# thu-ml/stochastic_gcn

Hardware: AMD Instinct MI355X
Metric: training edges/s (SpMM) (higher is better)
Workload: dtype f32

## Files before the change

include/sgcn.h:

```cpp
#ifndef SGCN_H
#define SGCN_H
#include <stdint.h>

#ifdef __cplusplus
extern "C" {
#endif

#define SGCN_OK 0
#define SGCN_ERR_INVALID (-1)
#define SGCN_ERR_HIP (-2)
#define SGCN_ERR_EMPTY_PROB (-3)
#define SGCN_ERR_NAN (-4)

const char* sgcn_last_error(void);
int sgcn_abi_version(void);


typedef struct { int32_t row, start, end, slot; } sgcn_seg_t;
typedef struct { int32_t row, first_slot, nslots; } sgcn_fix_t;
typedef struct {
    const sgcn_seg_t* dev_seg; int64_t nseg;
    const sgcn_fix_t* dev_fix; int64_t nfix;
    int64_t nslots;
    float* dev_ws;
// ... 59 lines not shown
                        int32_t* host_tile_rows, int32_t* host_tile_slots, sgcn_fix_t* host_fix);
void sgcn_csbuild_free(sgcn_csbuild_t* b);
int sgcn_cs_warp_table(const int32_t* host_col, int64_t nnz, int32_t K, int32_t max_buckets, int32_t mode,
                       double auto_dev, int32_t nthreads, uint32_t* host_table, int32_t* nbuckets, int32_t* shift);
int sgcn_csr_transpose_host(const int32_t* host_rowptr, const int32_t* host_col, const float* host_val, int32_t M,
                            int32_t K, int32_t nthreads, int32_t* host_t_rowptr, int32_t* host_t_col, float* host_t_val);
int32_t sgcn_host_threads(void);
int sgcn_reorder_lp(const int32_t* host_rowptr, const int32_t* host_col, int32_t n, int32_t max_iters,
                    uint32_t seed, int32_t min_size, int32_t* host_comm, int32_t* ncomm);
int sgcn_spmm_cs_f32(const sgcn_csplan_t* plan, int32_t M, int32_t K, int32_t d,
                     const float* dev_B, int64_t ldb, const int32_t* dev_gidx,
                     const float* dev_rscale, const float* dev_cscale,
                     float* dev_C, int64_t ldc, float beta, void* stream);

int sgcn_spmm_cs_variant(const sgcn_csplan_t* plan, int32_t d, char* buf, int32_t buflen);

typedef struct {
    int32_t VW, NW, RW, S, U;
    int32_t nparts;
    int32_t unit;
    int32_t xcd_tile_ptr[9];
    int64_t ntiles, nchunks, nent;
    const int32_t* dev_tile_chunk_ptr;
    const int32_t* dev_chunk_cols;
    const int32_t* dev_chunk_hdr;
    const int64_t* dev_ent_ptr;
    const uint32_t* dev_words;
    const float* dev_vals;
    const float* dev_row_fold;
    const int32_t* dev_tile_rows;
    const int32_t* dev_tile_slots;
    const sgcn_fix_t* dev_fix; int64_t nfix; int64_t nslots;
    float* dev_ws; int64_t ws_elems;
} sgcn_ldsplan_t;
typedef struct sgcn_ldsplan_host sgcn_ldsplan_host_t;
int sgcn_ldsplan_create(const int32_t* host_rowptr, const int32_t* host_col, const float* host_val,
                        int32_t M, int32_t K, const int32_t* host_col_pos, const int32_t* host_row_group,
                        int32_t VW, int32_t T, int32_t min_reuse, int32_t mode, int32_t ring_slots,
                        sgcn_ldsplan_host_t** out);
int sgcn_ldsplan_sizes(const sgcn_ldsplan_host_t* h, int64_t* sizes19);
int sgcn_ldsplan_export(const sgcn_ldsplan_host_t* h, int32_t* tile_chunk_ptr, int32_t* chunk_cols,
                        int32_t* chunk_hdr, int64_t* ent_ptr, uint32_t* words, float* vals, float* row_fold,
                        int32_t* tile_rows, int32_t* tile_slots, sgcn_fix_t* fix, int32_t* res_rowptr,
                        int32_t* res_col, float* res_val);
void sgcn_ldsplan_destroy(sgcn_ldsplan_host_t* h);
int sgcn_spmm_lds_f32(const sgcn_ldsplan_t* plan, int32_t M, int32_t K, int32_t d,
                      const float* dev_B, int64_t ldb, const float* dev_rscale,
                      float* dev_C, int64_t ldc, float beta, void* stream);

int sgcn_lds_profile_buffer(void* dev_buf);

int sgcn_tune(const char* key, int64_t value);
int64_t sgcn_tune_get(const char* key);

int sgcn_vr_aggregate_f32(const int32_t* dev_a_rowptr, const int32_t* dev_a_col,
                          const float* dev_a_val, const int32_t* dev_f_rowptr,
                          const int32_t* dev_f_col, const float* dev_f_val,
                          int32_t n1, int32_t n0, int32_t nf, int32_t d,
                          const float* dev_h, const float* dev_mu, int64_t ldx,
                          const float* dev_Hbar, int64_t ldh,
                          const int32_t* dev_ifield, const int32_t* dev_ffield,
                          const float* dev_s,
                          float* dev_out_h, float* dev_out_mu, int64_t ldo,
                          int32_t cvd, int32_t concat_self,
                          const sgcn_plan_t* f_plan ,
                          void* stream);

int sgcn_vr_aggregate_pre_f32(const int32_t* dev_f_rowptr, const int32_t* dev_f_col, const float* dev_f_val,
                              int32_t n1, int32_t nf, int32_t d, const float* dev_Hbar, int64_t ldh,
                              const int32_t* dev_ffield, float* dev_accP, const sgcn_plan_t* f_plan,
                              void* stream);
int sgcn_vr_aggregate_post_f32(const int32_t* dev_a_rowptr, const int32_t* dev_a_col, const float* dev_a_val,
                               int32_t n1, int32_t n0, int32_t d, const float* dev_h, const float* dev_mu,
                               int64_t ldx, const float* dev_Hbar, int64_t ldh, const int32_t* dev_ifield,
                               const float* dev_s, float* dev_out_h, float* dev_out_mu, int64_t ldo,
                               int32_t cvd, int32_t concat_self, const float* dev_accP, void* stream);

int sgcn_gather_rows_f32(const float* dev_in, int64_t ldi, const int32_t* dev_r, int32_t n,
                         int32_t d, float* dev_out, int64_t ldo, void* stream);

int sgcn_scatter_rows_f32(float* dev_H, int64_t ldh, const int32_t* dev_r, int32_t n,
                          int32_t d, const float* dev_src, int64_t lds, void* stream);

int sgcn_vr_aggregate_h16(const int32_t* dev_a_rowptr, const int32_t* dev_a_col,
                          const float* dev_a_val, const int32_t* dev_f_rowptr,
                          const int32_t* dev_f_col, const float* dev_f_val,
                          int32_t n1, int32_t n0, int32_t nf, int32_t d,
                          const float* dev_h, const float* dev_mu, int64_t ldx,
                          const uint16_t* dev_Hbar, int64_t ldh,
                          const int32_t* dev_ifield, const int32_t* dev_ffield,
                          const float* dev_s,
                          float* dev_out_h, float* dev_out_mu, int64_t ldo,
                          int32_t cvd, int32_t concat_self,
                          const sgcn_plan_t* f_plan, void* stream);
int sgcn_vr_aggregate_pre_h16(const int32_t* dev_f_rowptr, const int32_t* dev_f_col, const float* dev_f_val,
                              int32_t n1, int32_t nf, int32_t d, const uint16_t* dev_Hbar, int64_t ldh,
                              const int32_t* dev_ffield, float* dev_accP, const sgcn_plan_t* f_plan,
                              void* stream);
int sgcn_vr_aggregate_post_h16(const int32_t* dev_a_rowptr, const int32_t* dev_a_col, const float* dev_a_val,
                               int32_t n1, int32_t n0, int32_t d, const float* dev_h, const float* dev_mu,
                               int64_t ldx, const uint16_t* dev_Hbar, int64_t ldh, const int32_t* dev_ifield,
                               const float* dev_s, float* dev_out_h, float* dev_out_mu, int64_t ldo,
                               int32_t cvd, int32_t concat_self, const float* dev_accP, void* stream);
int sgcn_gather_rows_h16(const uint16_t* dev_H, int64_t ldh, const int32_t* dev_r, int32_t n,
                         int32_t d, float* dev_out, int64_t ldo, void* stream);
int sgcn_scatter_rows_h16(uint16_t* dev_H, int64_t ldh, const int32_t* dev_r, int32_t n,
// ... 301 lines not shown
```

stochastic_gcn_amd/_ffi.py:

```python
import ctypes as C
import os

import torch

_HERE = os.path.dirname(os.path.abspath(__file__))
LIB_PATH = os.path.join(_HERE, "libsgcn.so")

ABI_VERSION = 16

c_i32p = C.POINTER(C.c_int32)
c_f32p = C.POINTER(C.c_float)


class Seg(C.Structure):
    _fields_ = [("row", C.c_int32), ("start", C.c_int32), ("end", C.c_int32), ("slot", C.c_int32)]


class Fix(C.Structure):
    _fields_ = [("row", C.c_int32), ("first_slot", C.c_int32), ("nslots", C.c_int32)]


class CsPlan(C.Structure):
    _fields_ = [("R", C.c_int32), ("ntiles", C.c_int64), ("dev_tile_ptr", C.c_void_p),
                ("dev_colrow", C.c_void_p), ("dev_val", C.c_void_p), ("dev_tile_rows", C.c_void_p),
# ... 83 lines not shown
    "sgcn_spmm_lds_f32": (C.c_int, [C.POINTER(LdsPlan), C.c_int32, C.c_int32, C.c_int32, P, C.c_int64, P, P,
                                    C.c_int64, C.c_float, P]),
    "sgcn_vr_aggregate_f32": (C.c_int, [P, P, P, P, P, P, C.c_int32, C.c_int32, C.c_int32,
                                        C.c_int32, P, P, C.c_int64, P, C.c_int64, P, P, P, P, P,
                                        C.c_int64, C.c_int32, C.c_int32, C.POINTER(Plan), P]),
    "sgcn_vr_aggregate_pre_f32": (C.c_int, [P, P, P, C.c_int32, C.c_int32, C.c_int32, P, C.c_int64, P, P,
                                            C.POINTER(Plan), P]),
    "sgcn_vr_aggregate_post_f32": (C.c_int, [P, P, P, C.c_int32, C.c_int32, C.c_int32, P, P, C.c_int64, P, C.c_int64,
                                             P, P, P, P, C.c_int64, C.c_int32, C.c_int32, P, P]),
    "sgcn_gather_rows_f32": (C.c_int, [P, C.c_int64, P, C.c_int32, C.c_int32, P, C.c_int64, P]),
    "sgcn_scatter_rows_f32": (C.c_int, [P, C.c_int64, P, C.c_int32, C.c_int32, P, C.c_int64, P]),
    "sgcn_vr_aggregate_h16": (C.c_int, [P, P, P, P, P, P, C.c_int32, C.c_int32, C.c_int32,
                                        C.c_int32, P, P, C.c_int64, P, C.c_int64, P, P, P, P, P,
                                        C.c_int64, C.c_int32, C.c_int32, C.POINTER(Plan), P]),
    "sgcn_vr_aggregate_pre_h16": (C.c_int, [P, P, P, C.c_int32, C.c_int32, C.c_int32, P, C.c_int64, P, P,
                                            C.POINTER(Plan), P]),
    "sgcn_vr_aggregate_post_h16": (C.c_int, [P, P, P, C.c_int32, C.c_int32, C.c_int32, P, P, C.c_int64, P, C.c_int64,
                                             P, P, P, P, C.c_int64, C.c_int32, C.c_int32, P, P]),
    "sgcn_gather_rows_h16": (C.c_int, [P, C.c_int64, P, C.c_int32, C.c_int32, P, C.c_int64, P]),
    "sgcn_scatter_rows_h16": (C.c_int, [P, C.c_int64, P, C.c_int32, C.c_int32, P, C.c_int64, P]),
    "sgcn_hist_apply_h16": (C.c_int, [P, C.c_int64, P, C.c_int32, C.c_int32, C.c_int32, P, P]),
    "sgcn_spmm_csr_b16": (C.c_int, [P, P, P, C.c_int32, C.c_int32, C.c_int32, P, C.c_int64, P,
                                    P, P, P, C.c_int64, C.c_float, C.POINTER(Plan), P]),
    "sgcn_spmm_csr_add_b16": (C.c_int, [P, P, P, C.c_int32, C.c_int32, C.c_int32, P, C.c_int64, P,
                                        P, P, P, C.c_int64, C.c_float, C.POINTER(Plan), P, C.c_int64, C.c_int32, P]),
    "sgcn_spmm_cs_b16": (C.c_int, [C.POINTER(CsPlan), C.c_int32, C.c_int32, C.c_int32, P, C.c_int64, P,
                                   P, P, P, C.c_int64, C.c_float, P]),
    "sgcn_spmm_cs_variant_b16": (C.c_int, [C.POINTER(CsPlan), C.c_int32, C.c_char_p, C.c_int32]),
    "sgcn_coll_available": (C.c_int, [C.POINTER(C.c_int32)]),
    "sgcn_coll_retain": (C.c_int, []),
    "sgcn_coll_abort": (C.c_int, []),
    "sgcn_coll_async_error": (C.c_int, []),
    "sgcn_coll_unique_id": (C.c_int, [P]),
    "sgcn_coll_init": (C.c_int, [P, C.c_int32, C.c_int32]),
    "sgcn_coll_world": (C.c_int, []),
    "sgcn_coll_destroy": (C.c_int, []),
    "sgcn_coll_allreduce_avg_f32": (C.c_int, [P, C.c_int64, P]),
    "sgcn_coll_allgather_i32": (C.c_int, [P, P, C.c_int64, P]),
    "sgcn_coll_init_exchange": (C.c_int, [P]),
    "sgcn_coll_has_exchange": (C.c_int, []),
    "sgcn_coll_allgather_x_i32": (C.c_int, [P, P, C.c_int64, P]),
    "sgcn_hist_pack_f32": (C.c_int, [P, C.c_int32, P, C.c_int64, C.c_int32, C.c_int32, P, P]),
    "sgcn_hist_apply_f32": (C.c_int, [P, C.c_int64, P, C.c_int32, C.c_int32, C.c_int32, P, P]),
    "sgcn_csr_slice_indptr": (C.c_int, [C.c_int32, P, P, P]),
    "sgcn_csr_slice_indptr_dev": (C.c_int, [C.c_int32, P, P, P, P]),
    "sgcn_scale_rows_f32": (C.c_int, [P, C.c_int64, P, C.c_int32, C.c_int32, P, C.c_int64, P]),
    "sgcn_csr_slice_f32": (C.c_int, [C.c_int32, P, P, P, P, P, P, P, P, P]),
    "sgcn_ln_act_fwd_f32": (C.c_int, [P, C.c_int64, P, P, C.c_int32, C.c_int32, C.c_float, C.c_int32,
                                      P, C.c_int64, P, P, P]),
    "sgcn_ln_act_bwd_ws_floats": (C.c_int64, [C.c_int32, C.c_int32]),
    "sgcn_ln_act_bwd_f32": (C.c_int, [P, C.c_int64, P, C.c_int64, P, P, P, C.c_int32, C.c_int32,
                                      C.c_int32, P, C.c_int64, P, P, P, P]),
    "sgcn_gemm_ws_floats": (C.c_int64, [C.c_int32, C.c_int32, C.c_int32]),
    "sgcn_gemm_f32": (C.c_int, [C.c_int32, C.c_int32, C.c_int32, C.c_int32, C.c_int32, P, C.c_int64, P,
                                C.c_int64, P, C.c_int64, C.c_int32, P, P, P, P]),
    "sgcn_gemm_mb16_ws_floats": (C.c_int64, [C.c_int32, C.c_int32, C.c_int32, C.c_int32, C.c_int32]),
    "sgcn_gemm_mb16_f32": (C.c_int, [C.c_int32, C.c_int32, C.c_int32, C.c_int32, C.c_int32, P, C.c_int64, P,
                                     C.c_int64, P, C.c_int64, C.c_int32, P, P, P, P]),
    "sgcn_gemm_mb16_a16": (C.c_int, [C.c_int32, C.c_int32, C.c_int32, C.c_int32, C.c_int32, P, C.c_int64, P,
                                     C.c_int64, P, C.c_int64, C.c_int32, P, P, P, P]),
    "sgcn_dense_fwd_f32": (C.c_int, [C.c_int32, C.c_int32, C.c_int32, P, C.c_int64, P, C.c_int64, C.c_int32,
                                     P, C.c_int64, P, P, C.c_float, C.c_int32, P, C.c_int64, P, P, P, P, P, P, P]),
    "sgcn_dense_bwd_f32": (C.c_int, [C.c_int32, C.c_int32, C.c_int32, P, C.c_int64, P, C.c_int64, P, P, P,
                                     C.c_int32, P, C.c_int64, P, C.c_int64, P, C.c_int64, P, P, P, C.c_int64,
                                     P, P, P, P, P]),
    "sgcn_det_pre_f32": (C.c_int, [P, P, C.c_int64, C.c_float, P, P]),
    "sgcn_det_pre_bwd_f32": (C.c_int, [P, P, C.c_int64, C.c_float, P, P, P]),
    "sgcn_square_f32": (C.c_int, [P, C.c_int64, C.c_float, P, P]),
    "sgcn_addmul_f32": (C.c_int, [P, P, P, C.c_int64, C.c_float, P]),
    "sgcn_det_lnvar_fwd_f32": (C.c_int, [P, P, P, C.c_int32, C.c_int32, C.c_float, P, P]),
    "sgcn_det_lnvar_bwd_f32": (C.c_int, [P, P, P, P, P, C.c_int32, C.c_int32, C.c_float, P, P, P, P, P]),
    "sgcn_det_relu_fwd_f32": (C.c_int, [P, P, C.c_int64, P, P, P]),
    "sgcn_det_relu_bwd_f32": (C.c_int, [P, P, P, P, C.c_int64, P, P, P]),
    "sgcn_gauss_sample_f32": (C.c_int, [P, P, C.c_int64, C.c_uint32, P, P]),
    "sgcn_gauss_sample_bwd_f32": (C.c_int, [P, P, C.c_int64, C.c_uint32, P, P]),
    "sgcn_det_agg_prep_f32": (C.c_int, [P, P, P, P, C.c_int64, P, C.c_int32, C.c_int32, P, P, P, P, P, P]),
    "sgcn_det_agg_prep_bwd_f32": (C.c_int, [P, P, P, P, P, C.c_int32, C.c_int32, P, C.c_int64, C.c_int32, P, P]),
    "sgcn_relu_eps_f32": (C.c_int, [P, C.c_int64, C.c_int32, C.c_int32, C.c_float, P, C.c_int64, P]),
    "sgcn_gate_f32": (C.c_int, [P, C.c_int64, P, C.c_int64, C.c_int32, C.c_int32, P, P]),
    "sgcn_dropout_f32": (C.c_int, [P, C.c_int64, C.c_int32, C.c_int32, P, P, C.c_int64, P]),
    "sgcn_softmax_ce_f32": (C.c_int, [P, C.c_int64, P, C.c_int64, C.c_int32, C.c_int32, P, C.c_int64,
                                      P, C.c_int64, P, P, P]),
    "sgcn_sigmoid_ce_f32": (C.c_int, [P, C.c_int64, P, C.c_int64, C.c_int32, C.c_int32, P, C.c_int64,
                                      P, C.c_int64, P, P, P]),
    "sgcn_softmax_ce_rows_f32": (C.c_int, [P, C.c_int64, P, C.c_int64, C.c_int32, C.c_int32, P, C.c_int32, P, C.c_int64,
                                           P, C.c_int64, P, P, P]),
    "sgcn_sigmoid_ce_rows_f32": (C.c_int, [P, C.c_int64, P, C.c_int64, C.c_int32, C.c_int32, P, C.c_int32, P, C.c_int64,
                                           P, C.c_int64, P, P, P]),
    "sgcn_l2_penalty_f32": (C.c_int, [P, C.c_int64, C.c_int64, C.c_float, P, P, P]),
    "sgcn_csr_transpose_ws_ints": (C.c_int64, [C.c_int32, C.c_int64]),
    "sgcn_csr_transpose_index": (C.c_int, [C.c_int32, C.c_int64, P, P, P, P, P, P, P]),
    "sgcn_gather_f32": (C.c_int, [P, P, C.c_int64, P, P]),
    "sgcn_step_run": (C.c_int, [C.POINTER(StepOp), C.c_int32, P, C.c_int32, P]),
    "sgcn_step_fill": (C.c_int, [C.POINTER(StepFill), P, C.c_int64, C.c_int64, C.c_int64, C.c_int64, C.c_int64, C.c_float,
                                 P, C.c_int64]),
    "sgcn_copy_h2d_async": (C.c_int, [P, P, C.c_int64, P]),
    "sgcn_adam_f32": (C.c_int, [P, P, P, P, C.c_int64, C.c_float, C.c_float, C.c_float, C.c_float, P]),
    "sgcn_adam_ema_f32": (C.c_int, [P, P, P, P, P, C.c_int64, C.c_float, C.c_float, C.c_float, C.c_float, C.c_float, C.c_float, P]),
    "sgcn_moments_add_f32": (C.c_int, [P, C.c_int64, C.c_int64, P, P, P]),
    "sgcn_moments_summary_f64": (C.c_int, [P, P, C.c_int64, P, C.c_int64, P, P]),
    "sgcn_hist_error_ws_doubles": (C.c_int64, []),
    "sgcn_hist_error_f32": (C.c_int, [P, C.c_int64, P, C.c_int64, C.c_int64, C.c_int32, P, P, P]),
    "sgcn_hist_error_h16": (C.c_int, [P, C.c_int64, P, C.c_int64, C.c_int64, C.c_int32, P, P, P]),
    "sgcn_sched_create": (C.c_int, [P, P, P, C.c_int32, C.c_int32, C.c_int32, C.c_int32,
                                    C.c_int32, C.POINTER(C.c_void_p)]),
    "sgcn_sched_destroy": (None, [C.c_void_p]),
# ... 67 lines not shown
```

stochastic_gcn_amd/csrc/sgcn_agg.hip:

```cpp
#include "sgcn_dev.h"
#include <type_traits>

namespace sgcn {

int group_lanes(int nvec);

template <class HT>
struct AggArgsT {
    const int32_t* a_rowptr; const int32_t* a_col; const float* a_val;
    const int32_t* f_rowptr; const int32_t* f_col; const float* f_val;
    const sgcn_seg_t* seg; int64_t nseg; int64_t nsegblk;
    const float* h; const float* mu; int64_t ldx;
    const HT* H; int64_t ldh;
    const int32_t* ifield; const int32_t* ffield; const float* s;
    float* out_h; float* out_mu; int64_t ldo;
    int32_t d, nvec, cvd, off, concat;
    float* ws; int64_t ldw;
    int32_t pchunks;
    float* accP_out; const float* accP_in;
};


template <int VW>
__device__ __forceinline__ void store_masked(float* p, typename Vec<VW>::type v, int left) {
    if (left >= VW) vstore<VW>(p, v);
    else vstore_head<VW>(p, v, left);
}

template <int G, int VW, class HT>
__device__ __forceinline__ void agg_apart(const AggArgsT<HT>& a, int row, int vi, int lig, bool act,
                                          typename Vec<VW>::type& acc1, typename Vec<VW>::type& acc2) {
    typedef typename Vec<VW>::type VT;
    acc1 = vzero<VW>(); acc2 = vzero<VW>();
    const int start = uniform_i<G>(a.a_rowptr[row]), end = uniform_i<G>(a.a_rowptr[row + 1]);
    const int64_t voff = (int64_t)vi * VW;
    for (int p0 = start; p0 < end; p0 += G) {
        const int n = min(G, end - p0);
        int mycol = 0, myhist = 0;
        float myval = 0.f;
        if (lig < n) {
            mycol = a.a_col[p0 + lig];
            myval = a.a_val[p0 + lig];
            myhist = a.ifield[mycol];
        }
        for (int j = 0; j < n; j++) {
            const int c = bcast_i<G>(mycol, j);
            const int hr = bcast_i<G>(myhist, j);
            const float v = bcast_f<G>(myval, j);
            if (!act) continue;
            const VT hb = hload<VW>(a.H + (int64_t)hr * a.ldh + voff);
            const VT xv = vload<VW>(a.h + (int64_t)c * a.ldx + voff);
            if constexpr (VW == 1 && !std::is_same<HT, float>::value) {
                if (a.cvd) {
                    const float mv = a.mu[(int64_t)c * a.ldx + voff];
                    acc1 = __builtin_fmaf(v, mv - hb, acc1);
                    acc2 = __builtin_fmaf(v, xv - mv, acc2);
                } else {
                    acc1 = __builtin_fmaf(v, xv, acc1);
                    acc2 = __builtin_fmaf(v, hb, acc2);
                }
            } else if (a.cvd) {
                const VT mv = vload<VW>(a.mu + (int64_t)c * a.ldx + voff);
                acc1 += v * (mv - hb);
                acc2 += v * (xv - mv);
            } else {
                acc1 += v * xv;
                acc2 += v * hb;
            }
        }
    }
}

template <int VW, class HT>
__device__ __forceinline__ void agg_epilogue(const AggArgsT<HT>& a, int row, int vi, bool act, typename Vec<VW>::type accP,
                                             typename Vec<VW>::type acc1, typename Vec<VW>::type acc2) {
    typedef typename Vec<VW>::type VT;
    if (!act) return;
    const int64_t voff = (int64_t)vi * VW;
    const int left = a.d - vi * VW;
    float* oh = a.out_h + (int64_t)row * a.ldo;
    if (a.cvd) {
        float* om = a.out_mu + (int64_t)row * a.ldo;
        const VT mu_nbr = acc1 + accP;
        const VT h_nbr = acc2 * a.s[row] + mu_nbr;
        store_masked<VW>(oh + a.off + voff, h_nbr, left);
        store_masked<VW>(om + a.off + voff, mu_nbr, left);
        if (a.concat) {
            store_masked<VW>(oh + voff, vload<VW>(a.h + (int64_t)row * a.ldx + voff), left);
            store_masked<VW>(om + voff, vload<VW>(a.mu + (int64_t)row * a.ldx + voff), left);
        }
    } else {
        const VT out = (acc1 - acc2) + accP;
        store_masked<VW>(oh + a.off + voff, out, left);
        if (a.concat) store_masked<VW>(oh + voff, vload<VW>(a.h + (int64_t)row * a.ldx + voff), left);
    }
}

template <int G, int VW, class HT>
__device__ __forceinline__ void agg_finish(const AggArgsT<HT>& a, int row, int vi, int lig, bool act,
                                           typename Vec<VW>::type accP) {
    typename Vec<VW>::type acc1, acc2;
    agg_apart<G, VW>(a, row, vi, lig, act, acc1, acc2);
    agg_epilogue<VW>(a, row, vi, act, accP, acc1, acc2);
}

static int p_chunks(int32_t d, const void* Hbar, int64_t ldh, const float* ws) {
    const int vw = pick_vw(d, {Hbar, ws}, {ldh, ((int64_t)d + 3) / 4 * 4});
    return kBlock / group_lanes((d + vw - 1) / vw) - 1;
}

constexpr int agg_max_chunks(int G, int VW) { return (kBlock / G) * (4 / VW) - 1 < 31 ? (kBlock / G) * (4 / VW) - 1 : 31; }

template <int G, int VW, int U, class HT>
__global__ __launch_bounds__(kBlock) void agg_row_kernel(AggArgsT<HT> a) {
    typedef typename Vec<VW>::type VT;
    constexpr int NG = kBlock / G, NP = NG - 1;
    constexpr int NC = agg_max_chunks(G, VW);
    __shared__ float part[NC + 2][G * VW];
    const int lig = threadIdx.x & (G - 1), gq = threadIdx.x / G;
    const int slab = (int)(blockIdx.x / a.nseg);
    const int64_t s = blockIdx.x % a.nseg;
    int row, start, end, slot;
    if (a.seg) {
        const sgcn_seg_t sg = a.seg[s];
        row = sg.row; start = sg.start; end = sg.end; slot = sg.slot;
    } else {
        row = (int)s; start = a.f_rowptr[s]; end = a.f_rowptr[s + 1]; slot = -1;
    }
    row = uniform_i<G>(row); start = uniform_i<G>(start);
    end = uniform_i<G>(end); slot = uniform_i<G>(slot);
    const int vi = slab * G + lig;
    const bool act = vi < a.nvec;
    const bool finish_here = slot < 0 && !a.accP_out;
    const HT* Hl = a.H + (int64_t)vi * VW;

    const int nc = a.pchunks;
    if (gq < NP) {
        const int chunk = (end - start + nc - 1) / nc;
        for (int ck = gq; ck < nc; ck += NP) {
            const int gs = start + ck * chunk, ge = min(end, gs + chunk);
            VT accP = vzero<VW>();
            for (int p0 = gs; p0 < ge; p0 += G) {
                const int n = min(G, ge - p0);
                int myrow = 0;
                float myval = 0.f;
                if (lig < n) {
                    myrow = a.ffield[a.f_col[p0 + lig]];
                    myval = a.f_val[p0 + lig];
                }
                hpin<HT, VW>(myrow); hpin<HT, VW>(myval);
                for (int j = 0; j < n; j += U) {
                    typename HRaw<HT, VW>::type b[U];
                    float v[U];
#pragma unroll
                    for (int u = 0; u < U; u++) {
                        const bool in = j + u < n;
                        const int c = bcast_i<G>(myrow, in ? j + u : 0);
                        v[u] = in ? bcast_f<G>(myval, j + u) : 0.f;
                        b[u] = (act && in) ? hraw<VW>(Hl + (int64_t)c * a.ldh) : hraw_zero<HT, VW>();
                    }
#pragma unroll
                    for (int u = 0; u < U; u++) { hpin<HT, VW>(b[u]); accP += v[u] * hwiden<VW>(b[u]); }
                }
            }
            vstore<VW>(&part[ck][lig * VW], accP);
        }
    } else if (finish_here) {
        VT acc1, acc2;
        agg_apart<G, VW>(a, row, vi, lig, act, acc1, acc2);
        vstore<VW>(&part[NC][lig * VW], acc1);
        vstore<VW>(&part[NC + 1][lig * VW], acc2);
    }
    __syncthreads();
    if (gq != 0) return;
    VT accP = vload<VW>(&part[0][lig * VW]);
    if (nc == NP) {
#pragma unroll
        for (int q = 1; q < NP; q++) accP += vload<VW>(&part[q][lig * VW]);
    } else {
        for (int q = 1; q < nc; q++) accP += vload<VW>(&part[q][lig * VW]);
    }
    if (slot >= 0) { if (act) vstore<VW>(a.ws + (int64_t)slot * a.ldw + (int64_t)vi * VW, accP); }
    else if (a.accP_out) { if (act) vstore<VW>(a.accP_out + (int64_t)row * a.ldw + (int64_t)vi * VW, accP); }
    else agg_epilogue<VW>(a, row, vi, act, accP, vload<VW>(&part[NC][lig * VW]), vload<VW>(&part[NC + 1][lig * VW]));
}

template <int G, int VW, class HT>
__global__ __launch_bounds__(kBlock) void agg_fix_kernel(AggArgsT<HT> a, const sgcn_fix_t* fix, int64_t nfix) {
    typedef typename Vec<VW>::type VT;
    constexpr int GPB = kBlock / G;
    const int lig = threadIdx.x & (G - 1);
    const int64_t nfblk = (nfix + GPB - 1) / GPB;
    const int slab = (int)(blockIdx.x / nfblk);
    const int64_t f = (blockIdx.x % nfblk) * GPB + threadIdx.x / G;
    if (f >= nfix) return;
    const sgcn_fix_t fx = fix[f];
    const int vi = slab * G + lig;
    const bool act = vi < a.nvec;
    VT accP = vzero<VW>();
    if (act) {
        const float* w = a.ws + (int64_t)fx.first_slot * a.ldw + (int64_t)vi * VW;
        for (int q = 0; q < fx.nslots; q++) accP += vload<VW>(w + (int64_t)q * a.ldw);
    }
    if (a.accP_out) { if (act) vstore<VW>(a.accP_out + (int64_t)fx.row * a.ldw + (int64_t)vi * VW, accP); }
    else agg_finish<G, VW>(a, uniform_i<G>(fx.row), vi, lig, act, accP);
}

template <int G, int VW, class HT>
__global__ __launch_bounds__(kBlock) void agg_post_kernel(AggArgsT<HT> a, int32_t n1) {
    typedef typename Vec<VW>::type VT;
    constexpr int GPB = kBlock / G;
    const int lig = threadIdx.x & (G - 1);
    const int64_t nrblk = ((int64_t)n1 + GPB - 1) / GPB;
    const int slab = (int)(blockIdx.x / nrblk);
    const int64_t row = (blockIdx.x % nrblk) * GPB + threadIdx.x / G;
    if (row >= n1) return;
    const int vi = slab * G + lig;
    const bool act = vi < a.nvec;
    const VT accP = act ? vload<VW>(a.accP_in + row * a.ldw + (int64_t)vi * VW) : vzero<VW>();
    agg_finish<G, VW>(a, uniform_i<G>((int)row), vi, lig, act, accP);
}

template <int VW, class HT>
static int launch_agg_post(int G, const AggArgsT<HT>& a, int32_t n1, hipStream_t st) {
    const int nslab = (a.nvec + G - 1) / G;
#define SGCN_AGGP_CASE(GG)                                                                               \
    case GG: {                                                                                           \
        const int64_t nrblk = ((int64_t)n1 + (kBlock / GG) - 1) / (kBlock / GG);                          \
        hipLaunchKernelGGL((agg_post_kernel<GG, VW, HT>), dim3((unsigned)(nrblk * nslab)), dim3(kBlock), 0, st, a, n1); \
        break;                                                                                           \
    }
    switch (G) {
        SGCN_AGGP_CASE(8)
        SGCN_AGGP_CASE(16)
        SGCN_AGGP_CASE(32)
        SGCN_AGGP_CASE(64)
        default: return fail(SGCN_ERR_INVALID, "vr_aggregate_post: bad group %d", G);
    }
#undef SGCN_AGGP_CASE
    SGCN_HIP_TRY(hipGetLastError());
    return SGCN_OK;
}

template <int VW, class HT>
static int launch_agg(int G, const AggArgsT<HT>& a, const sgcn_plan_t* plan, hipStream_t st) {
    const int nslab = (a.nvec + G - 1) / G;
    SGCN_REQUIRE(a.pchunks >= 1 && a.pchunks <= agg_max_chunks(G, VW), "vr_aggregate: %d chunks of a P row, at most %d here",
                 a.pchunks, agg_max_chunks(G, VW));
    const int64_t nblocks = a.nseg * nslab;
    SGCN_REQUIRE(nblocks < (1ll << 31), "vr_aggregate: grid too large");
#define SGCN_AGG_CASE(GG)                                                                          \
    case GG: {                                                                                     \
        hipLaunchKernelGGL((agg_row_kernel<GG, VW, 16, HT>), dim3((unsigned)nblocks), dim3(kBlock), 0,  \
                           st, a);                                                                 \
        if (plan && plan->nfix > 0) {                                                              \
            const int64_t nfblk = (plan->nfix + (kBlock / GG) - 1) / (kBlock / GG);               \
            hipLaunchKernelGGL((agg_fix_kernel<GG, VW, HT>), dim3((unsigned)(nfblk * nslab)),          \
                               dim3(kBlock), 0, st, a, plan->dev_fix, plan->nfix);                 \
// ... 16 lines not shown

using namespace sgcn;

template <class HT>
static const void* vw_table(const HT* Hbar) { return std::is_same<HT, float>::value ? Hbar : nullptr; }

template <class HT>
static int vr_aggregate(const char* who, const int32_t* a_rowptr, const int32_t* a_col, const float* a_val,
                        const int32_t* f_rowptr, const int32_t* f_col, const float* f_val, int32_t n1, int32_t n0, int32_t nf,
                        int32_t d, const float* h, const float* mu, int64_t ldx, const HT* Hbar, int64_t ldh,
                        const int32_t* ifield, const int32_t* ffield, const float* s, float* out_h, float* out_mu, int64_t ldo,
                        int32_t cvd, int32_t concat_self, const sgcn_plan_t* f_plan, void* stream) {
    constexpr bool kH16 = !std::is_same<HT, float>::value;
    SGCN_REQUIRE(n1 >= 0 && n0 >= 0 && nf >= 0 && d >= 0, "%s: negative size", who);
    if constexpr (kH16) { if (int rc = h16_table_ok(who, Hbar, ldh, d)) return rc; }
    if (n1 == 0 || d == 0) return SGCN_OK;
    SGCN_REQUIRE(a_rowptr && f_rowptr && h && Hbar && ifield && out_h, "%s: null operand", who);
    SGCN_REQUIRE(nf == 0 || ffield, "%s: null ffield", who);
    SGCN_REQUIRE(!cvd || (mu && s && out_mu), "%s: cvd needs mu, s, out_mu", who);
    SGCN_REQUIRE(n1 <= n0 || !concat_self, "%s: concat_self needs n1 <= n0", who);
    const int64_t width = concat_self ? 2 * (int64_t)d : d;
    SGCN_REQUIRE(ldx >= d && ldh >= d && ldo >= width, "%s: leading dimension too small", who);

    AggArgsT<HT> a{};
    a.a_rowptr = a_rowptr; a.a_col = a_col; a.a_val = a_val;
    a.f_rowptr = f_rowptr; a.f_col = f_col; a.f_val = f_val;
    a.h = h; a.mu = mu; a.ldx = ldx; a.H = Hbar; a.ldh = ldh;
    a.ifield = ifield; a.ffield = ffield; a.s = s;
    a.out_h = out_h; a.out_mu = out_mu; a.ldo = ldo;
    a.d = d; a.cvd = cvd; a.concat = concat_self; a.off = concat_self ? d : 0;
    a.nseg = n1;
    if (f_plan) {
        SGCN_REQUIRE(f_plan->dev_seg && f_plan->nseg >= n1, "%s: malformed plan", who);
        a.seg = f_plan->dev_seg; a.nseg = f_plan->nseg;
        a.ws = f_plan->dev_ws; a.ldw = ((int64_t)d + 3) / 4 * 4;
        if (f_plan->nfix > 0) {
            SGCN_REQUIRE(f_plan->dev_fix && f_plan->dev_ws, "%s: plan needs dev_fix/dev_ws", who);
            SGCN_REQUIRE(f_plan->ws_elems >= f_plan->nslots * a.ldw, "%s: workspace too small", who);
        }
    }
    int vw = pick_vw(d, {h, mu, vw_table(Hbar), out_h, out_mu, f_plan ? f_plan->dev_ws : nullptr}, {ldx, ldh, ldo});
    if (concat_self) while (vw > 1 && d % vw != 0) vw >>= 1;
    a.nvec = (d + vw - 1) / vw;
    const int G = group_lanes(a.nvec);
    a.pchunks = p_chunks(d, vw_table(Hbar), ldh, f_plan ? f_plan->dev_ws : nullptr);
    a.nsegblk = (a.nseg + (kBlock / G) - 1) / (kBlock / G);
    hipStream_t st = (hipStream_t)stream;
    if (vw == 4) return launch_agg<4>(G, a, f_plan, st);
    if (vw == 2) return launch_agg<2>(G, a, f_plan, st);
    return launch_agg<1>(G, a, f_plan, st);
}

template <class HT>
static int vr_aggregate_pre(const char* who, const int32_t* f_rowptr, const int32_t* f_col, const float* f_val, int32_t n1,
                            int32_t nf, int32_t d, const HT* Hbar, int64_t ldh, const int32_t* ffield, float* accP,
                            const sgcn_plan_t* f_plan, void* stream) {
    constexpr bool kH16 = !std::is_same<HT, float>::value;
    SGCN_REQUIRE(n1 >= 0 && nf >= 0 && d >= 0, "%s: negative size", who);
    if constexpr (kH16) { if (int rc = h16_table_ok(who, Hbar, ldh, d)) return rc; }
    if (n1 == 0 || d == 0) return SGCN_OK;
    SGCN_REQUIRE(f_rowptr && Hbar && accP && ldh >= d, "%s: bad operand", who);
    SGCN_REQUIRE(nf == 0 || ffield, "%s: null ffield", who);
    AggArgsT<HT> a{};
    a.f_rowptr = f_rowptr; a.f_col = f_col; a.f_val = f_val;
    a.H = Hbar; a.ldh = ldh; a.ffield = ffield; a.d = d;
    a.ldw = ((int64_t)d + 3) / 4 * 4;
    a.accP_out = accP;
    a.nseg = n1;
    if (f_plan) {
        SGCN_REQUIRE(f_plan->dev_seg && f_plan->nseg >= n1, "%s: malformed plan", who);
        a.seg = f_plan->dev_seg; a.nseg = f_plan->nseg; a.ws = f_plan->dev_ws;
        if (f_plan->nfix > 0) {
            SGCN_REQUIRE(f_plan->dev_fix && f_plan->dev_ws, "%s: plan needs dev_fix/dev_ws", who);
            SGCN_REQUIRE(f_plan->ws_elems >= f_plan->nslots * a.ldw, "%s: workspace too small", who);
        }
    }
    const int vw = pick_vw(d, {vw_table(Hbar), accP, f_plan ? f_plan->dev_ws : nullptr}, {ldh, a.ldw});
    a.nvec = (d + vw - 1) / vw;
    const int G = group_lanes(a.nvec);
    a.pchunks = p_chunks(d, vw_table(Hbar), ldh, f_plan ? f_plan->dev_ws : nullptr);
    a.nsegblk = (a.nseg + (kBlock / G) - 1) / (kBlock / G);
    hipStream_t st = (hipStream_t)stream;
    if (vw == 4) return launch_agg<4>(G, a, f_plan, st);
    if (vw == 2) return launch_agg<2>(G, a, f_plan, st);
    return launch_agg<1>(G, a, f_plan, st);
}

template <class HT>
static int vr_aggregate_post(const char* who, const int32_t* a_rowptr, const int32_t* a_col, const float* a_val, int32_t n1,
                             int32_t n0, int32_t d, const float* h, const float* mu, int64_t ldx, const HT* Hbar, int64_t ldh,
                             const int32_t* ifield, const float* s, float* out_h, float* out_mu, int64_t ldo, int32_t cvd,
                             int32_t concat_self, const float* accP, void* stream) {
    constexpr bool kH16 = !std::is_same<HT, float>::value;
    SGCN_REQUIRE(n1 >= 0 && n0 >= 0 && d >= 0, "%s: negative size", who);
    if constexpr (kH16) { if (int rc = h16_table_ok(who, Hbar, ldh, d)) return rc; }
    if (n1 == 0 || d == 0) return SGCN_OK;
    SGCN_REQUIRE(a_rowptr && h && Hbar && ifield && out_h && accP, "%s: null operand", who);
    SGCN_REQUIRE(!cvd || (mu && s && out_mu), "%s: cvd needs mu, s, out_mu", who);
    SGCN_REQUIRE(n1 <= n0 || !concat_self, "%s: concat_self needs n1 <= n0", who);
    const int64_t width = concat_self ? 2 * (int64_t)d : d;
    SGCN_REQUIRE(ldx >= d && ldh >= d && ldo >= width, "%s: leading dimension too small", who);
    AggArgsT<HT> a{};
    a.a_rowptr = a_rowptr; a.a_col = a_col; a.a_val = a_val;
    a.h = h; a.mu = mu; a.ldx = ldx; a.H = Hbar; a.ldh = ldh; a.ifield = ifield; a.s = s;
    a.out_h = out_h; a.out_mu = out_mu; a.ldo = ldo;
    a.d = d; a.cvd = cvd; a.concat = concat_self; a.off = concat_self ? d : 0;
    a.ldw = ((int64_t)d + 3) / 4 * 4;
    a.accP_in = accP;
    int vw = pick_vw(d, {h, mu, vw_table(Hbar), out_h, out_mu, accP}, {ldx, ldh, ldo, a.ldw});
    if (concat_self) while (vw > 1 && d % vw != 0) vw >>= 1;
    a.nvec = (d + vw - 1) / vw;
    const int G = group_lanes(a.nvec);
    hipStream_t st = (hipStream_t)stream;
    if (vw == 4) return launch_agg_post<4>(G, a, n1, st);
    if (vw == 2) return launch_agg_post<2>(G, a, n1, st);
    return launch_agg_post<1>(G, a, n1, st);
}

extern "C" int sgcn_vr_aggregate_f32(const int32_t* a_rowptr, const int32_t* a_col, const float* a_val,
                                     const int32_t* f_rowptr, const int32_t* f_col, const float* f_val, int32_t n1,
                                     int32_t n0, int32_t nf, int32_t d, const float* h, const float* mu, int64_t ldx,
                                     const float* Hbar, int64_t ldh, const int32_t* ifield, const int32_t* ffield,
                                     const float* s, float* out_h, float* out_mu, int64_t ldo, int32_t cvd,
                                     int32_t concat_self, const sgcn_plan_t* f_plan, void* stream) {
    return vr_aggregate<float>("vr_aggregate", a_rowptr, a_col, a_val, f_rowptr, f_col, f_val, n1, n0, nf, d, h, mu, ldx, Hbar,
                               ldh, ifield, ffield, s, out_h, out_mu, ldo, cvd, concat_self, f_plan, stream);
}

extern "C" int sgcn_vr_aggregate_pre_f32(const int32_t* f_rowptr, const int32_t* f_col, const float* f_val, int32_t n1,
                                         int32_t nf, int32_t d, const float* Hbar, int64_t ldh, const int32_t* ffield,
                                         float* accP, const sgcn_plan_t* f_plan, void* stream) {
    return vr_aggregate_pre<float>("vr_aggregate_pre", f_rowptr, f_col, f_val, n1, nf, d, Hbar, ldh, ffield, accP, f_plan, stream);
}

extern "C" int sgcn_vr_aggregate_post_f32(const int32_t* a_rowptr, const int32_t* a_col, const float* a_val, int32_t n1,
                                          int32_t n0, int32_t d, const float* h, const float* mu, int64_t ldx,
                                          const float* Hbar, int64_t ldh, const int32_t* ifield, const float* s,
                                          float* out_h, float* out_mu, int64_t ldo, int32_t cvd, int32_t concat_self,
                                          const float* accP, void* stream) {
// ... 30 lines not shown
```

stochastic_gcn_amd/csrc/sgcn_fuse.h:

```cpp
#pragma once
#include <cstdint>
#include "../../include/sgcn.h"

namespace sgcn {

struct CeLastLayer {
    const float* W = nullptr; int64_t ldw = 0; int32_t K = 0;
    float* dx = nullptr; int64_t lddx = 0; const sgcn_dropout_t* dx_drop = nullptr;
    const float* hx = nullptr; int64_t ldhx = 0; int32_t kg = 1; const sgcn_dropout_t* h_drop = nullptr;
    bool pre = false;
    const float* px = nullptr; int64_t ldpx = 0; int32_t PK = 0; const float* PW = nullptr;
    int32_t pS = 1, pkchunk = 0, pkg = 1; const sgcn_dropout_t* p_drop = nullptr;
    const float* poff = nullptr; const float* psc = nullptr; float peps = 0.f; int32_t prelu = 0;
    float* pY = nullptr; int64_t ldpy = 0; float* pxhat = nullptr; float* prstd = nullptr;
};

}
```

stochastic_gcn_amd/csrc/sgcn_gemm.hip:

```cpp
#include "sgcn_dev.h"
#include "sgcn_bwd.h"

namespace sgcn {

typedef float f16acc __attribute__((ext_vector_type(16)));

constexpr int kTM = 32, kTN = 128, kTK = 32;

struct GemmArgs {
    const float* A; int64_t lda;
    const float* B; int64_t ldb;
    float* C; int64_t ldc;
    int32_t M, N, K;
    int32_t accumulate;
    int32_t kchunk;
    float* ws;
    const float* offset; const float* scale; float eps; int32_t relu;
    float* xhat; float* rstd;
    int32_t epi;
    const float* A2; int64_t lda2; int32_t a_split;
    DropArgs drop_a;
    DropArgs drop_c;
    int32_t vec_a, vec_b;
    const int32_t* a_gidx;
    const int32_t* a_gidx2;
};

__device__ __forceinline__ float wsum(float v) {
#pragma unroll
    for (int o = 32; o > 0; o >>= 1) v += __shfl_xor(v, o, 64);
    return v;
}

constexpr int kAsFloats = kTM * (kTK + 1), kBsFloats = kTK * (kTN + 4);
constexpr int kGroupFloats = kAsFloats + kBsFloats;

template <bool TA, bool TB, int KG>
__device__ __forceinline__ void gemm_body(const GemmArgs& g, const int bx, const int by, const int bz) {
    extern __shared__ float smem[];
    const int kg = threadIdx.x / kBlock;
    const int tid = threadIdx.x % kBlock, lane = tid & 63, wave = tid >> 6;
    float (*As)[kTK + 1] = reinterpret_cast<float (*)[kTK + 1]>(smem + kg * kGroupFloats);
    float (*Bs)[kTN + 4] = reinterpret_cast<float (*)[kTN + 4]>(smem + kg * kGroupFloats + kAsFloats);
    const int m0 = bx * kTM, n0 = by * kTN;
    const int kbeg = bz * g.kchunk;
    const int kend = min(g.K, kbeg + g.kchunk);
    f16acc acc = {};
    float ra[4], rb[16];
    float ep_scale[2] = {1.f, 1.f}, ep_offset[2] = {0.f, 0.f};
    if (g.epi == 2) {
#pragma unroll
        for (int e = 0; e < 2; e++) {
            const int c = (threadIdx.x & 63) + e * kWave;
            if (c < g.N) { ep_scale[e] = g.scale[c]; ep_offset[e] = g.offset[c]; }
// ... 121 lines not shown
#pragma unroll
        for (int r = 0; r < 16; r++) {
            const int row = m0 + (r & 3) + 8 * (r >> 2) + 4 * (lane >> 5), col = n0 + cj;
            if (row < g.M && col < g.N) {
                float* p = base + (int64_t)row * ld + col;
                float v = acc[r];
                if (g.drop_c.on) v *= drop_factor(g.drop_c, row, col);
                *p = add ? *p + v : v;
            }
        }
        return;
    }
    float (*Cs)[kTN + 4] = reinterpret_cast<float (*)[kTN + 4]>(smem + kAsFloats);
    if (KG > 1) __syncthreads();
    if (kg == 0) {
#pragma unroll
        for (int r = 0; r < 16; r++) Cs[(r & 3) + 8 * (r >> 2) + 4 * (lane >> 5)][cj] = acc[r];
    }
    __syncthreads();
    for (int rr = kg * (kBlock / kWave) + wave; rr < kTM; rr += KG * (kBlock / kWave)) {
        const int row = m0 + rr;
        if (row >= g.M) break;
        float* yr = g.C + (int64_t)row * g.ldc;
        if (g.epi == 1) {
            for (int c = lane; c < g.N; c += kWave) { const float v = Cs[rr][c]; yr[c] = g.relu ? fmaxf(v, 0.f) : v; }
            continue;
        }
        float s = 0.f;
        for (int c = lane; c < g.N; c += kWave) s += Cs[rr][c];
        const float mean = wsum(s) / (float)g.N;
        float q = 0.f;
        for (int c = lane; c < g.N; c += kWave) { const float t = Cs[rr][c] - mean; q += t * t; }
        const float rs = rsqrtf(wsum(q) / (float)g.N + g.eps);
        if (lane == 0) g.rstd[row] = rs;
        float* hr = g.xhat + (int64_t)row * g.N;
#pragma unroll
        for (int e = 0; e < 2; e++) {
            const int c = lane + e * kWave;
            if (c < g.N) {
                const float h = (Cs[rr][c] - mean) * rs;
                hr[c] = h;
                const float v = h * ep_scale[e] + ep_offset[e];
                yr[c] = g.relu ? fmaxf(v, 0.f) : v;
            }
        }
    }
}

template <bool TA, bool TB, int KG>
__global__ __launch_bounds__(kBlock * KG) void gemm_kernel(GemmArgs g) {
    gemm_body<TA, TB, KG>(g, (int)blockIdx.x, (int)blockIdx.y, (int)blockIdx.z);
}

struct GemmGroup {
    GemmArgs g[kMaxGroup];
    int32_t first[kMaxGroup + 1];
    int32_t gx[kMaxGroup], gy[kMaxGroup];
    int32_t n;
};

template <bool TA, bool TB, int KG>
__global__ __launch_bounds__(kBlock * KG) void gemm_group_kernel(GemmGroup G) {
    const int b = (int)blockIdx.x;
    int j = 0;
#pragma unroll
    for (int q = 1; q < kMaxGroup; q++) j += (q < G.n && b >= G.first[q]) ? 1 : 0;
    const int l = b - G.first[j];
    const int gx = G.gx[j], gy = G.gy[j];
    gemm_body<TA, TB, KG>(G.g[j], l % gx, (l / gx) % gy, l / (gx * gy));
}

__global__ void splitk_reduce_kernel(const float* __restrict__ ws, int32_t S, int32_t M, int32_t N,
                                     float* __restrict__ C, int64_t ldc, int32_t accumulate) {
    const int64_t i = (int64_t)blockIdx.x * blockDim.x + threadIdx.x;
    const int64_t mn = (int64_t)M * N;
    if (i >= mn) return;
    float s = 0.f;
    for (int z = 0; z < S; z++) s += ws[(int64_t)z * mn + i];
    float* p = C + (i / N) * ldc + (i % N);
    *p = accumulate ? *p + s : s;
}

__global__ void dense_bwd_reduce_kernel(ReduceJob j, int32_t gemm_blocks, const float* __restrict__ ln_partial,
                                        int32_t nblk, int32_t d, float* __restrict__ doffset,
                                        float* __restrict__ dscale, int32_t ln_accumulate) {
    if ((int)blockIdx.x < gemm_blocks) {
        const int64_t i = (int64_t)blockIdx.x * blockDim.x + threadIdx.x;
        const int64_t mn = (int64_t)j.M * j.N;
        if (i >= mn) return;
        float s = 0.f;
        for (int z = 0; z < j.S; z++) s += j.ws[(int64_t)z * mn + i];
        float* p = j.C + (i / j.N) * j.ldc + (i % j.N);
        *p = j.accumulate ? *p + s : s;
    } else {
        ln_param_reduce_cols32(ln_partial, nblk, d, doffset, dscale, (int)blockIdx.x - gemm_blocks, ln_accumulate != 0);
    }
}

__global__ void dense_bwd_reduce_multi_kernel(ReduceMulti R) { reduce_multi_body(R, (int)blockIdx.x, nullptr); }

__global__ __launch_bounds__(kBlock) void splitk_ln_act_kernel(const float* __restrict__ ws, int32_t S,
                                                               GemmArgs g) {
    const int lane = threadIdx.x & 63;
    const int64_t row = (int64_t)blockIdx.x * (kBlock / kWave) + threadIdx.x / kWave;
    if (row >= g.M) return;
    const int64_t mn = (int64_t)g.M * g.N;
    float v[2];
    float sc[2] = {1.f, 1.f}, of[2] = {0.f, 0.f};
    if (g.epi == 2) {
#pragma unroll
        for (int e = 0; e < 2; e++) {
            const int c = lane + e * kWave;
            if (c < g.N) { sc[e] = g.scale[c]; of[e] = g.offset[c]; }
        }
    }
#pragma unroll
    for (int e = 0; e < 2; e++) {
        const int c = lane + e * kWave;
        float s = 0.f;
        if (c < g.N)
            for (int z = 0; z < S; z++) s += ws[(int64_t)z * mn + row * g.N + c];
        v[e] = s;
    }
    float* yr = g.C + row * g.ldc;
    if (g.epi == 2) {
        const float mean = wsum(v[0] + v[1]) / (float)g.N;
        float q = 0.f;
#pragma unroll
        for (int e = 0; e < 2; e++) if (lane + e * kWave < g.N) { const float t = v[e] - mean; q += t * t; }
        const float rs = rsqrtf(wsum(q) / (float)g.N + g.eps);
        if (lane == 0) g.rstd[row] = rs;
#pragma unroll
        for (int e = 0; e < 2; e++) {
            const int c = lane + e * kWave;
            if (c < g.N) {
                const float h = (v[e] - mean) * rs;
                g.xhat[row * g.N + c] = h;
                const float y = h * sc[e] + of[e];
                yr[c] = g.relu ? fmaxf(y, 0.f) : y;
            }
        }
    } else {
#pragma unroll
        for (int e = 0; e < 2; e++) {
            const int c = lane + e * kWave;
            if (c < g.N) yr[c] = (g.epi == 1 && g.relu) ? fmaxf(v[e], 0.f) : v[e];
        }
    }
}


struct RowDense {
    const float* W; int64_t ldw; int32_t N, kg;
    const float* offset; const float* scale; float eps; int32_t relu, epi;
    DropArgs drop;
    float* Y; int64_t ldy; float* xhat; float* rstd;
};

__global__ __launch_bounds__(kBlock) void splitk_ln_dense_kernel(const float* __restrict__ ws, int32_t S, GemmArgs g, RowDense d) {
    extern __shared__ __attribute__((aligned(1024))) float wl[];
    const int lane = threadIdx.x & 63;
    const int64_t row = (int64_t)blockIdx.x * (kBlock / kWave) + threadIdx.x / kWave;
    const bool live = row < g.M;
    const int K2 = g.N, total = K2 * d.N;
    {
        const int total4 = total / 4, wave = threadIdx.x >> 6;
        for (int base4 = wave * kWave; base4 < total4; base4 += (kBlock / kWave) * kWave) {
            const int i4 = min(base4 + lane, total4 - 1);
            __builtin_amdgcn_global_load_lds((const __attribute__((address_space(1))) void*)(d.W + (int64_t)i4 * 4),
                                             (__attribute__((address_space(3))) void*)(wl + (int64_t)base4 * 4), 16, 0, 0);
        }
    }
    float sc1[2] = {1.f, 1.f}, of1[2] = {0.f, 0.f}, sc2[2] = {1.f, 1.f}, of2[2] = {0.f, 0.f};
#pragma unroll
    for (int e = 0; e < 2; e++) {
        const int c = lane + e * kWave;
        if (g.epi == 2 && c < g.N) { sc1[e] = g.scale[c]; of1[e] = g.offset[c]; }
        if (d.epi == 2 && c < d.N) { sc2[e] = d.scale[c]; of2[e] = d.offset[c]; }
    }
    const int64_t mn = (int64_t)g.M * g.N;
    float v[2] = {0.f, 0.f};
    if (live) {
#pragma unroll
        for (int e = 0; e < 2; e++) {
            const int c = lane + e * kWave;
            float s = 0.f;
            if (c < g.N)
                for (int z = 0; z < S; z++) s += ws[(int64_t)z * mn + row * g.N + c];
            v[e] = s;
        }
    }
    asm volatile("s_waitcnt vmcnt(0)" ::: "memory");
    __syncthreads();
    if (!live) return;
    float x[2];
    float* yr = g.C + row * g.ldc;
    if (g.epi == 2) {
        const float mean = wsum(v[0] + v[1]) / (float)g.N;
        float q = 0.f;
#pragma unroll
        for (int e = 0; e < 2; e++) if (lane + e * kWave < g.N) { const float t = v[e] - mean; q += t * t; }
        const float rs = rsqrtf(wsum(q) / (float)g.N + g.eps);
        if (lane == 0) g.rstd[row] = rs;
#pragma unroll
        for (int e = 0; e < 2; e++) {
            const int c = lane + e * kWave;
            x[e] = 0.f;
            if (c < g.N) {
                const float h = (v[e] - mean) * rs;
                g.xhat[row * g.N + c] = h;
                const float y = h * sc1[e] + of1[e];
                x[e] = g.relu ? fmaxf(y, 0.f) : y;
// ... 16 lines not shown
        const float xs = s0 < 2 ? x[0] : x[1];
        const int kb = s0 * 32, lb = kb & (kWave - 1);
        const float* wk = wl + kb * d.N;
        float p0 = a0[gi], p1 = a1[gi];
        if (kb + 32 <= K2) {
#pragma unroll
            for (int q = 0; q < 4; q++) {
                float w0[8], w1[8];
#pragma unroll
                for (int u = 0; u < 8; u++) { w0[u] = wk[(q * 8 + u) * d.N + c0]; w1[u] = wk[(q * 8 + u) * d.N + c1]; }
#pragma unroll
                for (int u = 0; u < 8; u++) {
                    const float xv = __int_as_float(__builtin_amdgcn_readlane(__float_as_int(xs), lb + q * 8 + u));
                    p0 = fmaf(xv, w0[u], p0); p1 = fmaf(xv, w1[u], p1);
                }
            }
        } else {
            for (int kk = 0; kb + kk < K2; kk++) {
                const float xv = __int_as_float(__builtin_amdgcn_readlane(__float_as_int(xs), lb + kk));
                p0 = fmaf(xv, wk[kk * d.N + c0], p0); p1 = fmaf(xv, wk[kk * d.N + c1], p1);
            }
        }
        a0[gi] = p0; a1[gi] = p1;
    }
    const float z[2] = {d.kg > 1 ? a0[0] + a0[1] : a0[0], d.kg > 1 ? a1[0] + a1[1] : a1[0]};
    float* y2 = d.Y + row * d.ldy;
    if (d.epi != 2) {
#pragma unroll
        for (int e = 0; e < 2; e++) {
            const int c = lane + e * kWave;
            if (c < d.N) y2[c] = (d.epi == 1 && d.relu) ? fmaxf(z[e], 0.f) : z[e];
        }
        return;
    }
    float s = 0.f;
#pragma unroll
    for (int e = 0; e < 2; e++) if (lane + e * kWave < d.N) s += z[e];
    const float mean = wsum(s) / (float)d.N;
    float q = 0.f;
#pragma unroll
    for (int e = 0; e < 2; e++) if (lane + e * kWave < d.N) { const float t = z[e] - mean; q += t * t; }
    const float rs = rsqrtf(wsum(q) / (float)d.N + d.eps);
    if (lane == 0) d.rstd[row] = rs;
#pragma unroll
    for (int e = 0; e < 2; e++) {
        const int c = lane + e * kWave;
        if (c < d.N) {
            const float h = (z[e] - mean) * rs;
            d.xhat[row * d.N + c] = h;
            const float y = h * sc2[e] + of2[e];
            y2[c] = d.relu ? fmaxf(y, 0.f) : y;
        }
    }
}

}

using namespace sgcn;

static int split_factor(int M, int N, int K) {
    const int tiles = ((M + kTM - 1) / kTM) * ((N + kTN - 1) / kTN);
    int s = 256 / std::max(tiles, 1);
    const int min_steps = tune_get("gemm_min_steps") > 0 ? tune_get("gemm_min_steps") : 3;
    s = std::min(s, K / (min_steps * kTK));
    return std::max(s, 1);
}

template <bool TA, bool TB, int KG>
static void launch_one(const GemmArgs& g, dim3 grid, hipStream_t st) {
    const size_t lds = (size_t)KG * kGroupFloats * sizeof(float);
    static bool raised = false;
    if (lds > 64 * 1024 && !raised) {
        (void)hipFuncSetAttribute(reinterpret_cast<const void*>(&gemm_kernel<TA, TB, KG>),
                                  hipFuncAttributeMaxDynamicSharedMemorySize, (int)lds);
        raised = true;
    }
    hipLaunchKernelGGL((gemm_kernel<TA, TB, KG>), grid, dim3(kBlock * KG), lds, st, g);
}

template <bool TA, bool TB>
static void launch_kg(const GemmArgs& g, dim3 grid, int kgroups, hipStream_t st) {
    if (kgroups >= 4) launch_one<TA, TB, 4>(g, grid, st);
    else if (kgroups == 2) launch_one<TA, TB, 2>(g, grid, st);
    else launch_one<TA, TB, 1>(g, grid, st);
}

struct GemmPlan { dim3 grid; int kgroups, S, epi; };

static GemmPlan prepare_gemm(GemmArgs& g, float* ws, int ta = 0, int tb = 0) {
    auto al = [](const void* p, int64_t ld) { return p && ((uintptr_t)p % 16 == 0) && (ld % 4 == 0); };
    g.vec_a = al(g.A, g.lda) && (!g.A2 || al(g.A2, g.lda2)) && (ta ? g.M : g.K) % 4 == 0;
    g.vec_b = al(g.B, g.ldb) && (tb ? g.K : g.N) % 4 == 0;
    int S = ws ? split_factor(g.M, g.N, g.K) : 1;
    g.kchunk = ((g.K + S - 1) / S + kTK - 1) / kTK * kTK;
    S = g.K > 0 ? (g.K + g.kchunk - 1) / g.kchunk : 1;
    if (g.K == 0) g.kchunk = kTK;
    g.ws = S > 1 ? ws : nullptr;
    GemmPlan p;
    p.epi = g.epi;
    p.S = S;
    if (S > 1) g.epi = 0;
    p.grid = dim3((unsigned)((g.M + kTM - 1) / kTM), (unsigned)((g.N + kTN - 1) / kTN), (unsigned)S);
    const int steps = (std::min(g.kchunk, g.K) + kTK - 1) / kTK;
    const int blocks = (int)(p.grid.x * p.grid.y * p.grid.z);
    p.kgroups = (blocks <= 128 && steps >= 8) ? 4 : ((blocks <= 256 && steps >= 4) ? 2 : 1);
    return p;
}

namespace sgcn {
void gemm_fwd_shape(int M, int N, int K, int* S, int* kgroups, int* kchunk) {
    GemmArgs g{};
    g.M = M; g.N = N; g.K = K;
    float dummy;
    const GemmPlan p = prepare_gemm(g, sgcn_gemm_ws_floats(M, N, K) > 0 ? &dummy : nullptr);
    *S = p.S; *kgroups = p.kgroups;
    if (kchunk) *kchunk = g.kchunk;
}
}

static void launch_prepared(const GemmArgs& g, const GemmPlan& p, int ta, int tb, hipStream_t st) {
    if (!ta && !tb) launch_kg<false, false>(g, p.grid, p.kgroups, st);
    else if (ta && !tb) launch_kg<true, false>(g, p.grid, p.kgroups, st);
    else if (!ta && tb) launch_kg<false, true>(g, p.grid, p.kgroups, st);
    else launch_kg<true, true>(g, p.grid, p.kgroups, st);
}

static int launch_gemm(GemmArgs g, int ta, int tb, float* ws, hipStream_t st, ReduceJob* defer = nullptr) {
    if (defer) defer->pending = 0;
    const GemmPlan p = prepare_gemm(g, ws, ta, tb);
    const int S = p.S, epi = p.epi;
    launch_prepared(g, p, ta, tb, st);
    if (S > 1 && epi != 0) {
        g.epi = epi;
        const unsigned rb = (unsigned)((g.M + (kBlock / kWave) - 1) / (kBlock / kWave));
        hipLaunchKernelGGL(splitk_ln_act_kernel, dim3(rb), dim3(kBlock), 0, st, g.ws, S, g);
    } else if (S > 1 && defer) {
        *defer = ReduceJob{g.ws, S, g.M, g.N, g.C, g.ldc, g.accumulate, 1};
    } else if (S > 1) {
        const int64_t mn = (int64_t)g.M * g.N;
        hipLaunchKernelGGL(splitk_reduce_kernel, dim3((unsigned)((mn + 255) / 256)), dim3(256), 0, st,
                           g.ws, S, g.M, g.N, g.C, g.ldc, g.accumulate);
    }
    SGCN_HIP_TRY(hipGetLastError());
    return SGCN_OK;
}

extern "C" int64_t sgcn_gemm_ws_floats(int32_t M, int32_t N, int32_t K) {
    if (M <= 0 || N <= 0 || K <= 0) return 0;
    const int S = split_factor(M, N, K);
    return S > 1 ? (int64_t)S * M * N : 0;
}

extern "C" int sgcn_gemm_f32(int32_t trans_a, int32_t trans_b, int32_t M, int32_t N, int32_t K,
                             const float* A, int64_t lda, const float* B, int64_t ldb, float* C,
                             int64_t ldc, int32_t accumulate, float* ws,
                             const sgcn_dropout_t* drop_a, const sgcn_dropout_t* drop_c, void* stream) {
    SGCN_REQUIRE(M >= 0 && N >= 0 && K >= 0, "gemm: negative size");
    if (M == 0 || N == 0) return SGCN_OK;
    SGCN_REQUIRE(C && (K == 0 || (A && B)), "gemm: null operand");
    GemmArgs g{};
    g.A = A; g.lda = lda; g.B = B; g.ldb = ldb; g.C = C; g.ldc = ldc;
    g.M = M; g.N = N; g.K = K; g.accumulate = accumulate; g.epi = 0;
    g.drop_a = drop_args(drop_a);
    g.drop_c = drop_args(drop_c);
    SGCN_REQUIRE(!g.drop_a.on || g.drop_a.width == (trans_a ? M : K), "gemm: drop_a width must be the stored A's row length");
    SGCN_REQUIRE(!g.drop_c.on || g.drop_c.width == N, "gemm: drop_c width must be N");
    if (g.drop_c.on) ws = nullptr;
    return launch_gemm(g, trans_a, trans_b, ws, (hipStream_t)stream);
}


namespace sgcn {
int dense_fwd_pair(int32_t M, int32_t N, int32_t K, const float* X, int64_t ldx, const float* X2, int64_t ldx2, int32_t split,
                   const float* W, int64_t ldw, const float* offset, const float* scale, float eps, int32_t relu, float* Y,
                   int64_t ldy, float* xhat, float* rstd, const sgcn_dropout_t* drop, float* ws, const int32_t* gidx,
                   const int32_t* gidx2, int32_t N2, const float* W2, int64_t ldw2, const float* offset2, const float* scale2,
                   float eps2, int32_t relu2, float* Y2, int64_t ldy2, float* xhat2, float* rstd2, const sgcn_dropout_t* drop2,
                   void* stream, int* fused) {
    *fused = 0;
    if (M <= 0 || N <= 0 || N > kTN || N2 <= 0 || N2 > kTN || !ws || !W2 || !Y2 || ldw2 != N2 || ldy != N) return SGCN_OK;
    const int norm = (offset && scale) ? 1 : 0, norm2 = (offset2 && scale2) ? 1 : 0;
    if ((norm && !(xhat && rstd)) || (norm2 && !(xhat2 && rstd2))) return SGCN_OK;
    GemmArgs g{};
    g.A = X; g.lda = ldx; g.B = W; g.ldb = ldw; g.C = Y; g.ldc = ldy;
    g.M = M; g.N = N; g.K = K; g.offset = offset; g.scale = scale; g.eps = eps; g.relu = relu;
    g.xhat = xhat; g.rstd = rstd; g.epi = norm ? 2 : (relu ? 1 : 0);
    g.A2 = X2; g.lda2 = ldx2; g.a_split = split;
    g.a_gidx = gidx; g.a_gidx2 = gidx2;
    g.drop_a = drop_args(drop);
    const GemmPlan p = prepare_gemm(g, ws);
    int S2 = 0, kg2 = 0;
    gemm_fwd_shape(M, N2, N, &S2, &kg2, nullptr);
    if (p.S <= 1 || S2 != 1 || kg2 > 2 || (size_t)N * N2 * sizeof(float) > 64 * 1024 || (N * N2) % 4 || !aligned16(W2)) return SGCN_OK;
    SGCN_REQUIRE(!g.drop_a.on || g.drop_a.width == K, "dense_fwd: dropout width must be K");
    RowDense d{};
    d.W = W2; d.ldw = ldw2; d.N = N2; d.kg = kg2; d.offset = offset2; d.scale = scale2; d.eps = eps2; d.relu = relu2;
    d.epi = norm2 ? 2 : (relu2 ? 1 : 0);
    d.drop = drop_args(drop2);
    SGCN_REQUIRE(!d.drop.on || d.drop.width == N, "dense_fwd: the second layer's dropout width must be its input width");
    d.Y = Y2; d.ldy = ldy2; d.xhat = xhat2; d.rstd = rstd2;
    hipStream_t st = (hipStream_t)stream;
    launch_prepared(g, p, 0, 0, st);
    g.epi = p.epi;
    const unsigned rb = (unsigned)((g.M + (kBlock / kWave) - 1) / (kBlock / kWave));
    hipLaunchKernelGGL(splitk_ln_dense_kernel, dim3(rb), dim3(kBlock), ((size_t)N * N2 + 255) / 256 * 256 * sizeof(float), st, g.ws, p.S, g, d);
    SGCN_HIP_TRY(hipGetLastError());
    *fused = 1;
    return SGCN_OK;
}
}

extern "C" int sgcn_dense_fwd_f32(int32_t M, int32_t N, int32_t K, const float* X, int64_t ldx,
                                  const float* X2, int64_t ldx2, int32_t split,
                                  const float* W, int64_t ldw, const float* offset,
                                  const float* scale, float eps, int32_t relu, float* Y, int64_t ldy,
                                  float* xhat, float* rstd, const sgcn_dropout_t* drop, float* ws,
                                  const int32_t* gidx, const int32_t* gidx2, void* stream) {
    SGCN_REQUIRE(M >= 0 && N >= 0 && K >= 0, "dense_fwd: negative size");
    if (M == 0 || N == 0) return SGCN_OK;
    SGCN_REQUIRE((X || (X2 && split == 0)) && W && Y, "dense_fwd: null operand");
    const int norm = (offset && scale) ? 1 : 0;
    SGCN_REQUIRE(!norm || (xhat && rstd), "dense_fwd: LayerNorm needs xhat / rstd");
    SGCN_REQUIRE(N <= kTN || (!norm && !relu), "dense_fwd: fused epilogue needs N <= 128");
    GemmArgs g{};
    g.A = X; g.lda = ldx; g.B = W; g.ldb = ldw; g.C = Y; g.ldc = ldy;
    g.M = M; g.N = N; g.K = K; g.offset = offset; g.scale = scale; g.eps = eps; g.relu = relu;
    g.xhat = xhat; g.rstd = rstd; g.epi = norm ? 2 : (relu ? 1 : 0);
    SGCN_REQUIRE(!X2 || (split >= 0 && split <= M), "dense_fwd: bad split");
    g.A2 = X2; g.lda2 = ldx2; g.a_split = split;
    g.a_gidx = gidx; g.a_gidx2 = gidx2;
    g.drop_a = drop_args(drop);
    SGCN_REQUIRE(!g.drop_a.on || g.drop_a.width == K, "dense_fwd: dropout width must be K");
    return launch_gemm(g, 0, 0, N <= kTN ? ws : nullptr, (hipStream_t)stream);
}


namespace sgcn {
namespace {
struct AuxCtx {
    hipStream_t st = nullptr;
    hipEvent_t fork = nullptr, join = nullptr;
    float* ring = nullptr;
    int64_t cap = 0, off = 0, want = 0;
    bool pending = false;
};
AuxCtx& aux_ctx() { static AuxCtx c; return c; }
int g_dw_recorded = 0;
int g_grad_store = 0;

int aux_init(AuxCtx& c) {
    if (c.st) return SGCN_OK;
    SGCN_HIP_TRY(hipStreamCreateWithFlags(&c.st, hipStreamNonBlocking));
    SGCN_HIP_TRY(hipEventCreateWithFlags(&c.fork, hipEventDisableTiming));
    SGCN_HIP_TRY(hipEventCreateWithFlags(&c.join, hipEventDisableTiming));
    return SGCN_OK;
}
}

int aux_fork(void* stream, void** aux_stream) {
// ... 300 lines not shown
```

stochastic_gcn_amd/csrc/sgcn_spmm.hip:

```cpp
#include "sgcn_dev.h"
#include <cstring>

namespace sgcn {

namespace {
int g_tune_nv = 0;
int g_tune_unroll = 0;
int g_tune_slabmajor = 1;
int g_tune_cs_round = 0;
int g_tune_cs_unroll = 0;
int g_tune_cs_pace = 0;
int g_tune_cs_slack = 0;
int g_tune_cs_noextra = 0;
int g_tune_step_overlap = 1;
int g_tune_step_fuse = 127;
int g_tune_cs_g2_wide = 0;
int g_tune_cs_nowarp = 0;
int g_tune_cs_last_pct = 80;
int g_tune_gemm_min_steps = 0;
int g_tune_gemm_mb16_slice_k = 0;
int g_tune_lds_wave_bias = 100;
int g_tune_lds_mix = 1;
int g_tune_lds_dbg = 0;
thread_local int tl_step_overlap = -1, tl_step_fuse = -1;
}

void step_mode_override(int overlap, int fuse) { tl_step_overlap = overlap; tl_step_fuse = fuse; }

int tune_get(const char* key) {
    if (!strcmp(key, "spmm_nv")) return g_tune_nv;
    if (!strcmp(key, "spmm_unroll")) return g_tune_unroll;
    if (!strcmp(key, "spmm_slabmajor")) return g_tune_slabmajor;
    if (!strcmp(key, "cs_round")) return g_tune_cs_round;
    if (!strcmp(key, "cs_unroll")) return g_tune_cs_unroll;
    if (!strcmp(key, "cs_pace")) return g_tune_cs_pace;
    if (!strcmp(key, "cs_slack")) return g_tune_cs_slack;
    if (!strcmp(key, "cs_noextra")) return g_tune_cs_noextra;
    if (!strcmp(key, "step_overlap")) return tl_step_overlap >= 0 ? tl_step_overlap : g_tune_step_overlap;
    if (!strcmp(key, "step_fuse")) return tl_step_fuse >= 0 ? tl_step_fuse : g_tune_step_fuse;
    if (!strcmp(key, "cs_g2_wide")) return g_tune_cs_g2_wide;
    if (!strcmp(key, "cs_nowarp")) return g_tune_cs_nowarp;
    if (!strcmp(key, "cs_last_pct")) return g_tune_cs_last_pct;
    if (!strcmp(key, "gemm_min_steps")) return g_tune_gemm_min_steps;
    if (!strcmp(key, "gemm_mb16_slice_k")) return g_tune_gemm_mb16_slice_k;
    if (!strcmp(key, "lds_wave_bias")) return g_tune_lds_wave_bias;
    if (!strcmp(key, "lds_mix")) return g_tune_lds_mix;
    if (!strcmp(key, "lds_dbg")) return g_tune_lds_dbg;
    return -1;
}

struct SpmmArgs {
    const int32_t* rowptr;
    const int32_t* col;
    const float* val;
    const sgcn_seg_t* seg;
    int64_t nseg;
    int64_t nsegblk;
    const void* B;
    int64_t ldb;
    const int32_t* gidx;
    const float* rscale;
    const float* cscale;
    float* C;
    int64_t ldc;
    float beta;
    int32_t d;
    int32_t nvec;
    float* ws;
    int64_t ldw;
    int32_t slabmajor;
    const float* add;
    int64_t ldadd;
    int32_t add_rows;
};

template <int VW>
__device__ __forceinline__ void epilogue_store(const SpmmArgs& a, int row, int vi,
                                               typename Vec<VW>::type acc, float rs) {
    float* out = a.C + (int64_t)row * a.ldc + (int64_t)vi * VW;
    typename Vec<VW>::type r = acc * rs;
    const int left = a.d - vi * VW;
    if (a.beta != 0.f) {
        if (left >= VW) r += a.beta * vload<VW>(out);
        else {
#pragma unroll
            for (int e = 0; e < VW; e++)
                if (e < left) {
                    if constexpr (VW == 1) r += a.beta * out[0]; else r[e] += a.beta * out[e];
                }
        }
    }
    if (a.add && row < a.add_rows) {
// ... 132 lines not shown
template <int VW, int U, class BT>
static bool dispatch_gnv(int G, int NV, const SpmmArgs& a, int64_t nblocks, hipStream_t st) {
    switch (G) {
        case 8: launch_seg<8, 1, VW, U, BT>(a, nblocks, st); return true;
        case 16: launch_seg<16, 1, VW, U, BT>(a, nblocks, st); return true;
        case 32: launch_seg<32, 1, VW, U, BT>(a, nblocks, st); return true;
        case 64:
            switch (NV) {
                case 1: launch_seg<64, 1, VW, U, BT>(a, nblocks, st); return true;
                case 2: launch_seg<64, 2, VW, U, BT>(a, nblocks, st); return true;
                case 3: launch_seg<64, 3, VW, U, BT>(a, nblocks, st); return true;
                case 4: launch_seg<64, 4, VW, U, BT>(a, nblocks, st); return true;
            }
    }
    return false;
}

template <int VW, class BT>
static bool dispatch_u(int U, int G, int NV, const SpmmArgs& a, int64_t nblocks, hipStream_t st) {
    switch (U) {
        case 2: return dispatch_gnv<VW, 2, BT>(G, NV, a, nblocks, st);
        case 4: return dispatch_gnv<VW, 4, BT>(G, NV, a, nblocks, st);
        case 8: return dispatch_gnv<VW, 8, BT>(G, NV, a, nblocks, st);
    }
    return false;
}

int group_lanes(int nvec) {
    if (nvec <= 8) return 8;
    if (nvec <= 16) return 16;
    if (nvec <= 32) return 32;
    return 64;
}

}

using namespace sgcn;

extern "C" int64_t sgcn_tune_get(const char* key) { return key ? tune_get(key) : -1; }

extern "C" int sgcn_tune(const char* key, int64_t value) {
    if (!key) return fail(SGCN_ERR_INVALID, "sgcn_tune: null key");
    if (!strcmp(key, "spmm_nv")) { SGCN_REQUIRE(value >= 0 && value <= 4, "spmm_nv in 0..4"); g_tune_nv = (int)value; return SGCN_OK; }
    if (!strcmp(key, "spmm_unroll")) {
        SGCN_REQUIRE(value == 0 || value == 2 || value == 4 || value == 8, "spmm_unroll in {0,2,4,8}");
        g_tune_unroll = (int)value; return SGCN_OK;
    }
    if (!strcmp(key, "spmm_slabmajor")) { g_tune_slabmajor = value != 0; return SGCN_OK; }
    if (!strcmp(key, "cs_pace")) { SGCN_REQUIRE(value >= 0, "cs_pace >= 0"); g_tune_cs_pace = (int)value; return SGCN_OK; }
    if (!strcmp(key, "cs_slack")) { SGCN_REQUIRE(value >= 0, "cs_slack >= 0"); g_tune_cs_slack = (int)value; return SGCN_OK; }
    if (!strcmp(key, "cs_noextra")) { g_tune_cs_noextra = value != 0; return SGCN_OK; }
    if (!strcmp(key, "step_overlap")) { g_tune_step_overlap = value != 0; return SGCN_OK; }
    if (!strcmp(key, "step_fuse")) { SGCN_REQUIRE(value >= 0 && value <= 127, "step_fuse in 0..127"); g_tune_step_fuse = (int)value; return SGCN_OK; }
    if (!strcmp(key, "cs_g2_wide")) { g_tune_cs_g2_wide = value != 0; return SGCN_OK; }
    if (!strcmp(key, "cs_nowarp")) { g_tune_cs_nowarp = value != 0; return SGCN_OK; }
    if (!strcmp(key, "gemm_min_steps")) { g_tune_gemm_min_steps = (int)value; return SGCN_OK; }
    if (!strcmp(key, "gemm_mb16_slice_k")) {
        SGCN_REQUIRE(value >= 0 && value <= 0x7fffffff, "gemm_mb16_slice_k >= 0");
        g_tune_gemm_mb16_slice_k = (int)value; return SGCN_OK;
    }
    if (!strcmp(key, "lds_wave_bias")) { SGCN_REQUIRE(value >= 50 && value <= 300, "lds_wave_bias in 50..300 (per cent)"); g_tune_lds_wave_bias = (int)value; return SGCN_OK; }
    if (!strcmp(key, "lds_mix")) { g_tune_lds_mix = value != 0; return SGCN_OK; }
    if (!strcmp(key, "lds_dbg")) { g_tune_lds_dbg = (int)value; return SGCN_OK; }
    if (!strcmp(key, "cs_last_pct")) { SGCN_REQUIRE(value >= 0 && value <= 100, "cs_last_pct in [0, 100]"); g_tune_cs_last_pct = (int)value; return SGCN_OK; }
    if (!strcmp(key, "cs_round")) { SGCN_REQUIRE(value >= 0, "cs_round >= 0"); g_tune_cs_round = (int)value; return SGCN_OK; }
    if (!strcmp(key, "cs_unroll")) {
        SGCN_REQUIRE(value == 0 || value == 4 || value == 8, "cs_unroll in {0,4,8}");
        g_tune_cs_unroll = (int)value; return SGCN_OK;
    }
    return fail(SGCN_ERR_INVALID, "sgcn_tune: unknown key '%s'", key);
}

template <class BT>
static int spmm_csr_add(const int32_t* rowptr, const int32_t* col, const float* val,
                        int32_t M, int32_t K, int32_t d, const BT* B, int64_t ldb,
                        const int32_t* gidx, const float* rscale, const float* cscale,
                        float* C, int64_t ldc, float beta, const sgcn_plan_t* plan,
                        const float* add, int64_t ldadd, int32_t add_rows, void* stream) {
    constexpr bool kB16 = !std::is_same<BT, float>::value;
    SGCN_REQUIRE(M >= 0 && K >= 0 && d >= 0, "spmm: negative size");
    if (M == 0 || d == 0) return SGCN_OK;
    SGCN_REQUIRE(rowptr && C && (B || K == 0), "spmm: null operand");
    SGCN_REQUIRE(ldb >= d && ldc >= d, "spmm: leading dimension smaller than d");
    if (kB16) {
        SGCN_REQUIRE(ldb % 8 == 0, "spmm: a bfloat16 operand needs ldb %% 8 == 0 (ldb %lld, d %d)", (long long)ldb, d);
        SGCN_REQUIRE(aligned16(B), "spmm: a bfloat16 operand needs a 16-byte aligned base");
    }
    hipStream_t st = (hipStream_t)stream;

    SpmmArgs a{};
    a.rowptr = rowptr; a.col = col; a.val = val;
    a.B = B; a.ldb = ldb; a.gidx = gidx; a.rscale = rscale; a.cscale = cscale;
    a.C = C; a.ldc = ldc; a.beta = beta; a.d = d;
    a.nseg = M;
    a.slabmajor = g_tune_slabmajor;
    if (add && add_rows > 0) {
        SGCN_REQUIRE(ldadd >= d && add_rows <= M, "spmm: bad addend");
        a.add = add; a.ldadd = ldadd; a.add_rows = add_rows;
    }
    if (plan) {
        SGCN_REQUIRE(plan->dev_seg && plan->nseg >= M, "spmm: malformed plan");
        a.seg = plan->dev_seg; a.nseg = plan->nseg;
        a.ws = plan->dev_ws; a.ldw = ((int64_t)d + 3) / 4 * 4;
        if (plan->nfix > 0) {
            SGCN_REQUIRE(plan->dev_fix && plan->dev_ws, "spmm: plan with split rows needs dev_fix/dev_ws");
            SGCN_REQUIRE(plan->ws_elems >= plan->nslots * a.ldw,
// ... 76 lines not shown
```

stochastic_gcn_amd/csrc/sgcn_step.cpp:

```cpp
#include <hip/hip_runtime_api.h>

#include <algorithm>
#include <chrono>
#include <cstdio>
#include <cstdlib>
#include <cstring>
#include <mutex>

#include "sgcn_host.h"
#include "sgcn_fuse.h"
#include "sgcn_bwd.h"
#include "../../include/sgcn.h"

namespace sgcn {
int dense_bwd_overlapped(int32_t n, int32_t N, int32_t K, const float* dy, int64_t lddy, const float* y, int64_t ldy,
                         const float* xhat, const float* rstd, const float* scale, int32_t relu, const float* x,
                         int64_t ldx, const float* W, int64_t ldw, float* dW, int64_t lddw, float* doffset,
                         float* dscale, float* dx, int64_t lddx, const sgcn_dropout_t* drop, float* g_tmp, float* ws,
                         const int32_t* gidx, void* stream);
int aux_join(void* stream);
void step_mode_override(int overlap, int fuse);
int dense_bwd_chain(const DenseBwdArgs& up, const DenseBwdArgs& lo, void* stream);
int aux_fork(void* stream, void** aux_stream);
int spin_launch(void* stream, int64_t usec);
int dw_group_begin();
int dw_group_flush(void* stream, bool park_reduce);
int reduce_flush(void* stream);
void dw_group_abort();
void grad_store_mode(int on);
void stats_defer(int on);
int stats_flush(void* stream);
int adam_with_stats(float* theta, const float* grad, float* m, float* v, int64_t n, float lr_t, float beta1, float beta2,
                    float eps, float* avg, float decay, float one_minus, void* stream);
bool scatter_park(float* H, int64_t ldh, const int32_t* idx, int32_t n, int32_t d, const float* src, int64_t lds);
int ce_impl(bool softmax, const float* logits, int64_t ldz, const float* labels, int64_t ldl, int32_t n, int32_t c,
            float* dlogits, int64_t lddz, float* pred, int64_t ldp, float* stats, float* rowstat, void* stream, bool overlap,
            const CeLastLayer* last);
void gemm_fwd_shape(int M, int N, int K, int* S, int* kgroups, int* kchunk);
int dense_fwd_pair(int32_t M, int32_t N, int32_t K, const float* X, int64_t ldx, const float* X2, int64_t ldx2, int32_t split,
                   const float* W, int64_t ldw, const float* offset, const float* scale, float eps, int32_t relu, float* Y,
                   int64_t ldy, float* xhat, float* rstd, const sgcn_dropout_t* drop, float* ws, const int32_t* gidx,
                   const int32_t* gidx2, int32_t N2, const float* W2, int64_t ldw2, const float* offset2, const float* scale2,
                   float eps2, int32_t relu2, float* Y2, int64_t ldy2, float* xhat2, float* rstd2, const sgcn_dropout_t* drop2,
                   void* stream, int* fused);
}

namespace {

inline float f32(int64_t v) {
    const uint32_t b = (uint32_t)(uint64_t)v;
    float f;
    std::memcpy(&f, &b, 4);
    return f;
}
template <class T> inline T* ptr(int64_t v) { return reinterpret_cast<T*>((uintptr_t)v); }

struct Args {
    int64_t v[SGCN_STEP_MAX_ARGS];
    int n, pos;
    int64_t next() { return pos < n ? v[pos++] : 0; }
    template <class T> T* p() { return ptr<T>(next()); }
    int32_t i() { return (int32_t)next(); }
    float f() { return f32(next()); }
    const sgcn_dropout_t* drop(sgcn_dropout_t* st) {
        const int64_t on = next();
        st->key = (uint32_t)next(); st->keep = f(); st->rows = i(); st->width = i();
        return on ? st : nullptr;
    }
    const sgcn_plan_t* plan(sgcn_plan_t* st) {
        const int64_t on = next();
        st->dev_seg = p<const sgcn_seg_t>(); st->nseg = next();
        st->dev_fix = p<const sgcn_fix_t>(); st->nfix = next();
        st->nslots = next(); st->dev_ws = p<float>(); st->ws_elems = next();
        if (st->nfix == 0) st->dev_fix = nullptr;
        return on ? st : nullptr;
    }
};


struct DenseFwdOp {
    int32_t M, N, K, split, relu; float eps;
    const float *X, *X2, *W, *off, *sc; int64_t ldx, ldx2, ldw, ldy, ws_cap;
    float *Y, *xhat, *rstd, *ws; const int32_t *g1, *g2;
    sgcn_dropout_t dr; bool has_drop;
    void read(Args& a) {
        M = a.i(); N = a.i(); K = a.i();
        X = a.p<const float>(); ldx = a.next(); X2 = a.p<const float>(); ldx2 = a.next(); split = a.i();
        W = a.p<const float>(); ldw = a.next(); off = a.p<const float>(); sc = a.p<const float>();
        eps = a.f(); relu = a.i();
        Y = a.p<float>(); ldy = a.next(); xhat = a.p<float>(); rstd = a.p<float>();
        has_drop = a.drop(&dr) != nullptr;
        ws = a.p<float>(); ws_cap = a.next(); g1 = a.p<const int32_t>(); g2 = a.p<const int32_t>();
    }
    const sgcn_dropout_t* drop() const { return has_drop ? &dr : nullptr; }
    bool plain() const { return !off && !sc && !relu; }
};
struct DenseBwdOp {
    int32_t n, N, K, relu;
    const float *dy, *y, *xhat, *rstd, *sc, *x, *W; int64_t lddy, ldy, ldx, ldw, lddw, lddx, ws_cap;
    float *dW, *doff, *dsc, *dx, *gtmp, *ws; const int32_t* gidx;
    sgcn_dropout_t dr; bool has_drop;
    void read(Args& a) {
        n = a.i(); N = a.i(); K = a.i();
        dy = a.p<const float>(); lddy = a.next(); y = a.p<const float>(); ldy = a.next();
        xhat = a.p<const float>(); rstd = a.p<const float>(); sc = a.p<const float>(); relu = a.i();
        x = a.p<const float>(); ldx = a.next(); W = a.p<const float>(); ldw = a.next();
        dW = a.p<float>(); lddw = a.next(); doff = a.p<float>(); dsc = a.p<float>();
        dx = a.p<float>(); lddx = a.next();
        has_drop = a.drop(&dr) != nullptr;
        gtmp = a.p<float>(); ws = a.p<float>(); ws_cap = a.next(); gidx = a.p<const int32_t>();
    }
    const sgcn_dropout_t* drop() const { return has_drop ? &dr : nullptr; }
};
struct CeOp {
    const float *z, *lab; int64_t ldz, ldl, lddz, ldp; int32_t n, c; float *dz, *pred, *stats, *rowstat;
    void read(Args& a) {
        z = a.p<const float>(); ldz = a.next(); lab = a.p<const float>(); ldl = a.next(); n = a.i(); c = a.i();
        dz = a.p<float>(); lddz = a.next(); pred = a.p<float>(); ldp = a.next(); stats = a.p<float>(); rowstat = a.p<float>();
    }
};
inline bool is_adam(int32_t op) { return op == SGCN_OP_ADAM || op == SGCN_OP_ADAM_EMA; }
constexpr int32_t f32_op(int32_t op) {
    return op == SGCN_OP_VR_AGG_H16 ? SGCN_OP_VR_AGG : op == SGCN_OP_VR_AGG_PRE_H16 ? SGCN_OP_VR_AGG_PRE
         : op == SGCN_OP_VR_AGG_POST_H16 ? SGCN_OP_VR_AGG_POST : op == SGCN_OP_SCATTER_ROWS_H16 ? SGCN_OP_SCATTER_ROWS
         : op == SGCN_OP_AUX_SCATTER_ROWS_H16 ? SGCN_OP_AUX_SCATTER_ROWS : op == SGCN_OP_HIST_APPLY_H16 ? SGCN_OP_HIST_APPLY : op;
}
inline bool is_ce(int32_t op) { return op == SGCN_OP_SOFTMAX_CE || op == SGCN_OP_SIGMOID_CE; }

}

extern "C" int sgcn_step_fill(const sgcn_step_fill_t* f, const int64_t* meta, int64_t meta_len, int64_t ip, int64_t fp,
                              int64_t seed, int64_t step, float lr, int64_t* slots, int64_t nslots) {
    if (!f || !meta || !slots || meta_len < 0 || nslots < 0 || f->n < 0 || f->n_cap < 0 || f->n_ws < 0 || f->n_keys < 0 ||
        f->n > nslots || f->lr_slot < 0 || f->lr_slot >= nslots || (f->n > 0 && (!f->idx || !f->mul || !f->base)) ||
        (f->n_cap > 0 && (!f->cap_idx || !f->cap_max)) || (f->n_ws > 0 && (!f->ws_idx || !f->ws_ld)) ||
        (f->n_keys > 0 && (!f->key_slot || !f->key_layer)))
        return sgcn::fail(SGCN_ERR_INVALID, "step_fill: bad argument");
    auto in_meta = [&](int64_t i) { return i >= 0 && i < meta_len; };
    for (int64_t j = 0; j < f->n_cap; j++) {
        if (!in_meta(f->cap_idx[j])) return sgcn::fail(SGCN_ERR_INVALID, "step_fill: capacity check outside the descriptor table");
        if (meta[f->cap_idx[j]] > f->cap_max[j]) return 1;
    }
    for (int64_t j = 0; j < f->n_ws; j++) {
        if (!in_meta(f->ws_idx[j])) return sgcn::fail(SGCN_ERR_INVALID, "step_fill: workspace check outside the descriptor table");
        if (meta[f->ws_idx[j]] * f->ws_ld[j] > f->ws_floats) return 1;
    }
    for (int64_t i = 0; i < f->n; i++)
        if (!in_meta(f->idx[i])) return sgcn::fail(SGCN_ERR_INVALID, "step_fill: slot %lld reads outside the descriptor table", (long long)i);
    for (int64_t j = 0; j < f->n_keys; j++)
        if (f->key_slot[j] < 0 || f->key_slot[j] >= nslots) return sgcn::fail(SGCN_ERR_INVALID, "step_fill: key slot out of range");
    for (int64_t i = 0; i < f->n; i++)
        slots[i] = meta[f->idx[i]] * f->mul[i] + (f->base[i] == 1 ? ip : f->base[i] == 2 ? fp : 0);
    auto fmix32 = [](uint32_t h) { h ^= h >> 16; h *= 0x85EBCA6Bu; h ^= h >> 13; h *= 0xC2B2AE35u; h ^= h >> 16; return h; };
    for (int64_t j = 0; j < f->n_keys; j++) {
        const uint32_t site = fmix32((uint32_t)seed * 0x9E3779B1u + (uint32_t)f->key_layer[j] * 0x85EBCA77u + 0x27D4EB2Fu);
        slots[f->key_slot[j]] = (int64_t)fmix32(site + (uint32_t)step * 0xC2B2AE3Du);
    }
    uint32_t bits;
    memcpy(&bits, &lr, sizeof(bits));
    slots[f->lr_slot] = (int64_t)bits;
    return SGCN_OK;
}

extern "C" int sgcn_copy_h2d_async(void* dst, const void* src, int64_t bytes, void* stream) {
    if (bytes < 0 || (bytes > 0 && (!dst || !src))) return sgcn::fail(SGCN_ERR_INVALID, "copy_h2d_async: bad argument");
    if (bytes == 0) return SGCN_OK;
// ... 41 lines not shown
        }
        SGCN_XCHG_TRY(hipStreamSynchronize((hipStream_t)stream));
        SGCN_XCHG_TRY(hipStreamSynchronize(cand[n]));
    }
    for (int i = 0; i < n; i++)
        if (i != got) (void)hipStreamDestroy(cand[i]);
    (void)hipEventDestroy(ev);
    c.st = got >= 0 ? cand[got] : nullptr;
    if (getenv("SGCN_XCHG_DEBUG")) fprintf(stderr, "sgcn: exchange stream: candidate %d of %d runs beside the step's stream\n", got, n);
    return SGCN_OK;
}

int xchg_fork(void* stream, void** side) {
    XchgCtx& c = xchg_ctx();
    if (!c.tried) {
        const int rc = xchg_pick(stream, c);
        if (rc != SGCN_OK) return rc;
        const unsigned flags = hipEventDisableTiming | (getenv("SGCN_XCHG_SYSFENCE") ? 0u : hipEventDisableSystemFence);
        SGCN_XCHG_TRY(hipEventCreateWithFlags(&c.fork, flags));
        SGCN_XCHG_TRY(hipEventCreateWithFlags(&c.done, flags));
    }
    if (!c.st) { *side = stream; return SGCN_OK; }
    if (!c.pending) {
        static const char* skip = getenv("SGCN_XCHG_DROPS_A_DEPENDENCY") ? getenv("SGCN_XCHG_SKIP") : nullptr;
        if (!(skip && strstr(skip, "fork"))) {
            SGCN_XCHG_TRY(hipEventRecord(c.fork, (hipStream_t)stream));
            SGCN_XCHG_TRY(hipStreamWaitEvent(c.st, c.fork, 0));
        }
        c.pending = true;
    }
    *side = (void*)c.st;
    return SGCN_OK;
}

int xchg_join(void* stream) {
    XchgCtx& c = xchg_ctx();
    if (!c.pending) return SGCN_OK;
    c.pending = false;
    static const char* skip = getenv("SGCN_XCHG_DROPS_A_DEPENDENCY") ? getenv("SGCN_XCHG_SKIP") : nullptr;
    if (skip && strstr(skip, "join")) return SGCN_OK;
    SGCN_XCHG_TRY(hipEventRecord(c.done, c.st));
    SGCN_XCHG_TRY(hipStreamWaitEvent((hipStream_t)stream, c.done, 0));
    return SGCN_OK;
}
}

extern "C" int sgcn_step_run(const sgcn_step_op_t* ops, int32_t nops, const int64_t* slots, int32_t nslots,
                             void* stream) {
    if (nops < 0 || (nops > 0 && !ops) || nslots < 0 || (nslots > 0 && !slots))
        return sgcn::fail(SGCN_ERR_INVALID, "step_run: bad argument");
    static std::mutex run_mutex;
    std::lock_guard<std::mutex> run_lock(run_mutex);
    bool memset_on_aux = false;
    int64_t run_overlap = sgcn_tune_get("step_overlap"), run_fuse = sgcn_tune_get("step_fuse");
    bool own_mode = false;
    for (int32_t k = 0; k < nops; k++)
        if (ops[k].op == SGCN_OP_MODE && ops[k].nargs >= 1) {
            own_mode = true;
            run_overlap = ops[k].add[0] != 0;
            if (ops[k].nargs >= 2 && ops[k].add[1] >= 0) run_fuse = ops[k].add[1] & 127;
        }
    const bool overlap = run_overlap != 0;
    const int fuse = (int)run_fuse;
    struct ModeGuard {
        bool on;
        ~ModeGuard() { if (on) sgcn::step_mode_override(-1, -1); }
    } mode{own_mode};
    if (own_mode) sgcn::step_mode_override(overlap ? 1 : 0, fuse);
    bool grouped = false, store = false, l2 = false;
    int ce_at = -1, adam_at = -1;
    for (int32_t k = 0; k < nops; k++) {
        grouped = grouped || ops[k].op == SGCN_OP_DW_FLUSH;
        store = store || ops[k].op == SGCN_OP_GRAD_STORE;
        l2 = l2 || ops[k].op == SGCN_OP_L2_PENALTY;
        if (ops[k].op == SGCN_OP_SOFTMAX_CE || ops[k].op == SGCN_OP_SIGMOID_CE) ce_at = k;
        if (is_adam(ops[k].op)) adam_at = k;
    }
    const bool park_stats = store && ce_at >= 0 && adam_at > ce_at && !l2;
    if (grouped) sgcn::dw_group_begin();
    sgcn::grad_store_mode(store ? 1 : 0);
    sgcn::stats_defer(park_stats ? 1 : 0);
    struct Guard {
        bool on; void* st;
        ~Guard() { if (on) sgcn::dw_group_abort(); sgcn::grad_store_mode(0); sgcn::stats_defer(0); sgcn::reduce_flush(st); sgcn::stats_flush(st); }
    } guard{grouped, stream};
    auto eval_args = [&](const sgcn_step_op_t& o, Args& a) {
        a.n = o.nargs; a.pos = 0;
        for (int j = 0; j < o.nargs; j++) {
            const int32_t s = o.slot[j];
            if (s >= nslots) return false;
            a.v[j] = (s < 0 ? 0 : o.mul[j] * slots[s]) + o.add[j];
        }
        return true;
    };
    int32_t skip_until = 0, dx_done_at = -1;
    struct Head { bool on = false, pre = false; int32_t at = -1, kg = 1, pS = 1, pkchunk = 0, pkg = 1; DenseFwdOp f, p; } head;
    auto peek = [&](int32_t j, Args& b) {
        return j < nops && ops[j].nargs >= 0 && ops[j].nargs <= SGCN_STEP_MAX_ARGS && eval_args(ops[j], b);
    };
    for (int32_t k = 0; k < nops; k++) {
        const sgcn_step_op_t& op = ops[k];
        if (op.nargs < 0 || op.nargs > SGCN_STEP_MAX_ARGS)
            return sgcn::fail(SGCN_ERR_INVALID, "step_run: op %d has %d arguments", k, op.nargs);
        if (k < skip_until) continue;
        Args a;
        if (!eval_args(ops[k], a)) return sgcn::fail(SGCN_ERR_INVALID, "step_run: op %d reads a slot beyond %d", k, nslots);
        int rc = SGCN_OK;
        sgcn_dropout_t dr;
        sgcn_plan_t pl;
        const int32_t base = f32_op(op.op);
        const bool h16 = base != op.op;
        if (is_adam(op.op) || base == SGCN_OP_L2_PENALTY || base == SGCN_OP_SCATTER_ROWS || base == SGCN_OP_MEMSET0 ||
            base == SGCN_OP_VR_AGG_POST || (base == SGCN_OP_DENSE_BWD && memset_on_aux)) {
            rc = sgcn::aux_join(stream);
            if (rc != SGCN_OK) return rc;
            memset_on_aux = false;
        }
        void* side = stream;
        if (overlap && (base == SGCN_OP_VR_AGG_PRE || base == SGCN_OP_AUX_SCATTER_ROWS || base == SGCN_OP_AUX_MEMSET0)) {
            rc = sgcn::aux_fork(stream, &side);
            if (rc != SGCN_OK) return rc;
        }
        auto fork_to = [&](int64_t where) {
            return where == 0 ? (int)SGCN_OK : where == 2 ? xchg_fork(stream, &side) : sgcn::aux_fork(stream, &side);
        };
        switch (op.op) {
        case SGCN_OP_DENSE_FWD: {
            DenseFwdOp f;
            f.read(a);
            head.on = false;
            Args b;
            if ((fuse & 1) && f.plain() && !f.X2 && !f.g1 && f.N <= 64 && f.K <= 128 && (int64_t)f.K * f.N * 4 <= 48 * 1024 &&
                peek(k + 1, b) && is_ce(ops[k + 1].op)) {
                CeOp ce;
                ce.read(b);
                int S = 0, kgq = 0;
                sgcn::gemm_fwd_shape(f.M, f.N, f.K, &S, &kgq, nullptr);
                if (S == 1 && kgq <= 2 && ce.z == f.Y && ce.ldz == f.ldy && ce.n == f.M && ce.c == f.N) {
                    head.on = true; head.pre = false; head.at = k + 1; head.kg = kgq; head.f = f;
                    break;
                }
            }
            if ((fuse & 16) && (fuse & 1) && !f.X2 && !f.g1 && f.N <= 128 && f.K <= 256 && (f.K * f.N) % 4 == 0 &&
                peek(k + 1, b) && ops[k + 1].op == SGCN_OP_DENSE_FWD && k + 2 < nops && is_ce(ops[k + 2].op)) {
                DenseFwdOp q;
                q.read(b);
                Args c3;
                CeOp ce;
                int S = 0, kgq = 0, S0 = 0, kg0 = 0, kc0 = 0;
                sgcn::gemm_fwd_shape(q.M, q.N, q.K, &S, &kgq, nullptr);
                sgcn::gemm_fwd_shape(f.M, f.N, f.K, &S0, &kg0, &kc0);
                const bool ok = q.plain() && !q.X2 && !q.g1 && q.N <= 64 && q.K == f.N && q.M == f.M && q.X == f.Y && q.ldx == f.ldy &&
                                (int64_t)q.K * q.N * 4 <= 48 * 1024 && S == 1 && kgq <= 2 && S0 >= 1 && S0 <= 2 && kg0 <= 2 &&
                                f.ldw == f.N && q.ldw == q.N && peek(k + 2, c3);
                if (ok) {
                    ce.read(c3);
                    if (ce.z == q.Y && ce.ldz == q.ldy && ce.n == q.M && ce.c == q.N &&
                        (((int64_t)q.K * q.N + 255) / 256 * 256 + ((int64_t)f.K * f.N + 255) / 256 * 256) * 4 <= 160 * 1024) {
                        head.on = true; head.pre = true; head.at = k + 2; head.kg = kgq; head.f = q; head.p = f;
                        head.pS = S0; head.pkchunk = kc0; head.pkg = kg0;
                        skip_until = k + 2;
                        break;
                    }
                }
            }
            const int64_t need = f.N <= 128 ? sgcn_gemm_ws_floats(f.M, f.N, f.K) : 0;
            if (need > f.ws_cap) return sgcn::fail(SGCN_ERR_INVALID, "step_run: GEMM scratch %lld > %lld floats", (long long)need, (long long)f.ws_cap);
            if ((fuse & 4) && need > 0 && peek(k + 1, b) && ops[k + 1].op == SGCN_OP_DENSE_FWD) {
                DenseFwdOp q;
                q.read(b);
                const bool is_head = (fuse & 1) && q.plain() && !q.X2 && q.N <= 64 && k + 2 < nops && is_ce(ops[k + 2].op);
                const bool whole = !is_head && q.X == f.Y && q.ldx == f.ldy && !q.g1 && !q.g2 && q.M == f.M && q.K == f.N &&
                                   (!q.X2 || (q.X2 == f.Y + (int64_t)q.split * f.ldy && q.ldx2 == f.ldy)) &&
                                   (!q.has_drop || q.dr.rows == q.split || !q.X2);
                if (whole) {
                    int fusedq = 0;
                    rc = sgcn::dense_fwd_pair(f.M, f.N, f.K, f.X, f.ldx, f.X2, f.ldx2, f.split, f.W, f.ldw, f.off, f.sc, f.eps, f.relu,
                                              f.Y, f.ldy, f.xhat, f.rstd, f.drop(), f.ws, f.g1, f.g2, q.N, q.W, q.ldw, q.off, q.sc, q.eps,
                                              q.relu, q.Y, q.ldy, q.xhat, q.rstd, q.drop(), stream, &fusedq);
                    if (rc != SGCN_OK) break;
                    if (fusedq) { skip_until = k + 2; break; }
                }
            }
            rc = sgcn_dense_fwd_f32(f.M, f.N, f.K, f.X, f.ldx, f.X2, f.ldx2, f.split, f.W, f.ldw, f.off, f.sc, f.eps, f.relu, f.Y, f.ldy,
                                    f.xhat, f.rstd, f.drop(), need ? f.ws : nullptr, f.g1, f.g2, stream);
            break;
        }
        case SGCN_OP_DENSE_BWD: {
            DenseBwdOp w;
            w.read(a);
            const bool norm = w.xhat != nullptr;
            const int64_t need = (norm ? (sgcn_ln_act_bwd_ws_floats(w.n, w.N) + 3) / 4 * 4 : 0) +
                                 std::max(sgcn_gemm_ws_floats(w.K, w.N, w.n), sgcn_gemm_ws_floats(w.n, w.K, w.N));
            if (need > w.ws_cap) return sgcn::fail(SGCN_ERR_INVALID, "step_run: backward scratch %lld > %lld floats", (long long)need, (long long)w.ws_cap);
            Args b;
            if ((fuse & 64) && w.dx && k != dx_done_at && peek(k + 1, b) && ops[k + 1].op == SGCN_OP_DENSE_BWD) {
                DenseBwdOp q;
                q.read(b);
                const bool qnorm = q.xhat != nullptr;
                const int64_t need2 = (qnorm ? (sgcn_ln_act_bwd_ws_floats(q.n, q.N) + 3) / 4 * 4 : 0) +
                                      std::max(sgcn_gemm_ws_floats(q.K, q.N, q.n), sgcn_gemm_ws_floats(q.n, q.K, q.N));
                if (q.dy == w.dx && q.lddy == w.lddx && q.n == w.n && q.N == w.K && !q.dx && need2 <= q.ws_cap) {
                    const sgcn::DenseBwdArgs up{w.n, w.N, w.K, w.dy, w.lddy, w.y, w.ldy, w.xhat, w.rstd, w.sc, w.relu, w.x, w.ldx, w.W, w.ldw,
                                                w.dW, w.lddw, w.doff, w.dsc, w.dx, w.lddx, w.drop(), w.gtmp, need ? w.ws : nullptr, w.gidx};
                    const sgcn::DenseBwdArgs lo{q.n, q.N, q.K, q.dy, q.lddy, q.y, q.ldy, q.xhat, q.rstd, q.sc, q.relu, q.x, q.ldx, q.W, q.ldw,
                                                q.dW, q.lddw, q.doff, q.dsc, nullptr, q.lddx, q.drop(), q.gtmp, need2 ? q.ws : nullptr, q.gidx};
                    rc = sgcn::dense_bwd_chain(up, lo, stream);
                    skip_until = k + 2;
                    break;
                }
            }
            rc = sgcn::dense_bwd_overlapped(w.n, w.N, w.K, w.dy, w.lddy, w.y, w.ldy, w.xhat, w.rstd, w.sc, w.relu, w.x, w.ldx, w.W, w.ldw,
                                            w.dW, w.lddw, w.doff, w.dsc, k == dx_done_at ? nullptr : w.dx, w.lddx, w.drop(), w.gtmp,
                                            need ? w.ws : nullptr, w.gidx, stream);
            break;
        }
        case SGCN_OP_DW_FLUSH:
            rc = sgcn::dw_group_flush(stream, (fuse & 32) && k + 1 < nops && is_adam(ops[k + 1].op));
            break;
        case SGCN_OP_GRAD_STORE:
        case SGCN_OP_MODE:
            break;
        case SGCN_OP_CSR_SLICE: {
            const int32_t n = a.i(); const int32_t* rows = a.p<const int32_t>();
            const float* av = a.p<const float>(); const int32_t* ac = a.p<const int32_t>(); const int32_t* arp = a.p<const int32_t>();
            int32_t* o_p = a.p<int32_t>(); float* o_d = a.p<float>(); int32_t* o_c = a.p<int32_t>(); int32_t* o_r = a.p<int32_t>();
            rc = sgcn_csr_slice_indptr_dev(n, rows, arp, o_p, stream);
            if (rc == SGCN_OK) rc = sgcn_csr_slice_f32(n, rows, av, ac, arp, o_p, o_d, o_c, o_r, stream);
            break;
        }
        case SGCN_OP_LN_ACT_FWD: {
            const float* x = a.p<const float>(); const int64_t ldx = a.next();
// ... 84 lines not shown
            break;
        }
        case SGCN_OP_GAUSS_BWD: {
            const float* var = a.p<const float>(); const float* g = a.p<const float>(); const int64_t n = a.next();
            const uint32_t key = (uint32_t)a.next(); float* d_var = a.p<float>();
            rc = sgcn_gauss_sample_bwd_f32(var, g, n, key, d_var, stream);
            break;
        }
        case SGCN_OP_DET_AGG_PREP: {
            const float* mu = a.p<const float>(); const float* var = a.p<const float>();
            const float* Hm = a.p<const float>(); const float* Hv = a.p<const float>(); const int64_t ldh = a.next();
            const int32_t* ifield = a.p<const int32_t>(); const int32_t n0 = a.i(), d = a.i();
            float* dmu = a.p<float>(); float* ds2 = a.p<float>(); float* msig2 = a.p<float>(); float* ds = a.p<float>(); float* sbar = a.p<float>();
            rc = sgcn_det_agg_prep_f32(mu, var, Hm, Hv, ldh, ifield, n0, d, dmu, ds2, msig2, ds, sbar, stream);
            break;
        }
        case SGCN_OP_DET_AGG_PREP_BWD: {
            const float* var = a.p<const float>(); const float* ds = a.p<const float>(); const float* sbar = a.p<const float>();
            const float* g_ds2 = a.p<const float>(); const float* g_msig2 = a.p<const float>(); const int32_t n0 = a.i(), d = a.i();
            const float* add = a.p<const float>(); const int64_t ldadd = a.next(); const int32_t add_rows = a.i(); float* d_var = a.p<float>();
            rc = sgcn_det_agg_prep_bwd_f32(var, ds, sbar, g_ds2, g_msig2, n0, d, add, ldadd, add_rows, d_var, stream);
            break;
        }
        case SGCN_OP_RELU_EPS: {
            const float* raw = a.p<const float>(); const int64_t ldr = a.next(); const int32_t n = a.i(), d = a.i();
            const float eps = a.f(); float* y = a.p<float>(); const int64_t ldy = a.next();
            rc = sgcn_relu_eps_f32(raw, ldr, n, d, eps, y, ldy, stream);
            break;
        }
        case SGCN_OP_GATE: {
            const float* raw = a.p<const float>(); const int64_t ldr = a.next();
            const float* g = a.p<const float>(); const int64_t ldg = a.next(); const int32_t n = a.i(), d = a.i(); float* out = a.p<float>();
            rc = sgcn_gate_f32(raw, ldr, g, ldg, n, d, out, stream);
            break;
        }
        case SGCN_OP_CSR_TRANSPOSE: {
            const int32_t ncols = a.i(); const int64_t nnz = a.next();
            const int32_t* col = a.p<const int32_t>(); const int32_t* row = a.p<const int32_t>();
            int32_t* trp = a.p<int32_t>(); int32_t* trow = a.p<int32_t>(); int32_t* tsrc = a.p<int32_t>();
            int32_t* ws = a.p<int32_t>(); const int64_t ws_cap = a.next();
            if (sgcn_csr_transpose_ws_ints(ncols, nnz) > ws_cap)
                return sgcn::fail(SGCN_ERR_INVALID, "step_run: transpose scratch too small at op %d", k);
            rc = sgcn_csr_transpose_index(ncols, nnz, col, row, trp, trow, tsrc, ws, stream);
            break;
        }
        case SGCN_OP_GATHER_F32: {
            const float* src = a.p<const float>(); const int32_t* idx = a.p<const int32_t>(); const int64_t n = a.next();
            float* out = a.p<float>();
            rc = sgcn_gather_f32(src, idx, n, out, stream);
            break;
        }
        case SGCN_OP_VR_AGG:
        case SGCN_OP_VR_AGG_H16: {
            const int32_t* arp = a.p<const int32_t>(); const int32_t* ac = a.p<const int32_t>(); const float* av = a.p<const float>();
            const int32_t* frp = a.p<const int32_t>(); const int32_t* fc = a.p<const int32_t>(); const float* fv = a.p<const float>();
            const int32_t n1 = a.i(), n0 = a.i(), nf = a.i(), d = a.i();
            const float* h = a.p<const float>(); const float* mu = a.p<const float>(); const int64_t ldx = a.next();
            const void* H = a.p<const void>(); const int64_t ldh = a.next();
            const int32_t* ifi = a.p<const int32_t>(); const int32_t* ffi = a.p<const int32_t>();
            const float* s = a.p<const float>();
            float* oh = a.p<float>(); float* om = a.p<float>(); const int64_t ldo = a.next();
            const int32_t cvd = a.i(), concat = a.i();
            const sgcn_plan_t* p = a.plan(&pl);
            rc = h16 ? sgcn_vr_aggregate_h16(arp, ac, av, frp, fc, fv, n1, n0, nf, d, h, mu, ldx, (const uint16_t*)H, ldh, ifi, ffi,
                                             s, oh, om, ldo, cvd, concat, p, stream)
                     : sgcn_vr_aggregate_f32(arp, ac, av, frp, fc, fv, n1, n0, nf, d, h, mu, ldx, (const float*)H, ldh, ifi, ffi,
                                             s, oh, om, ldo, cvd, concat, p, stream);
            break;
        }
        case SGCN_OP_SPMM: {
            const int32_t* rp = a.p<const int32_t>(); const int32_t* c = a.p<const int32_t>(); const float* v = a.p<const float>();
            const int32_t M = a.i(), K = a.i(), d = a.i();
            const float* B = a.p<const float>(); const int64_t ldb = a.next();
            const int32_t* gidx = a.p<const int32_t>(); const float* rs = a.p<const float>(); const float* cs = a.p<const float>();
            float* C = a.p<float>(); const int64_t ldc = a.next(); const float beta = a.f();
            const sgcn_plan_t* p = a.plan(&pl);
            const float* add = a.p<const float>(); const int64_t ldadd = a.next(); const int32_t add_rows = a.i();
            rc = add ? sgcn_spmm_csr_add_f32(rp, c, v, M, K, d, B, ldb, gidx, rs, cs, C, ldc, beta, p, add, ldadd, add_rows, stream)
                     : sgcn_spmm_csr_f32(rp, c, v, M, K, d, B, ldb, gidx, rs, cs, C, ldc, beta, p, stream);
            break;
        }
        case SGCN_OP_SOFTMAX_CE:
        case SGCN_OP_SIGMOID_CE: {
            CeOp ce;
            ce.read(a);
            const bool hd = head.on && head.at == k;
            DenseBwdOp t{};
            bool tail = false;
            Args b;
            if ((fuse & 2) && ce.dz && ce.c <= 64 && peek(k + 1, b) && ops[k + 1].op == SGCN_OP_DENSE_BWD) {
                t.read(b);
                tail = t.n == ce.n && t.N == ce.c && t.dy == ce.dz && t.lddy == ce.lddz && !t.xhat && !t.sc && !t.relu && t.dx && t.W &&
                       t.K > 0 && (int64_t)t.K * ce.c * 4 <= 48 * 1024 &&
                       (!hd || (t.W == head.f.W && t.K == head.f.K && t.ldw == head.f.ldw));
                if (tail) dx_done_at = k + 1;
            }
            sgcn::CeLastLayer L;
            if (hd || tail) {
                L.W = hd ? head.f.W : t.W; L.ldw = hd ? head.f.ldw : t.ldw; L.K = hd ? head.f.K : t.K;
            }
            if (tail) { L.dx = t.dx; L.lddx = t.lddx; L.dx_drop = t.drop(); }
            if (hd) {
                L.hx = head.pre ? nullptr : head.f.X; L.ldhx = head.f.ldx; L.kg = head.kg; L.h_drop = head.f.drop();
                if (head.pre) {
                    const DenseFwdOp& p = head.p;
                    L.pre = true; L.px = p.X; L.ldpx = p.ldx; L.PK = p.K; L.PW = p.W; L.pS = head.pS; L.pkchunk = head.pkchunk;
                    L.pkg = head.pkg; L.p_drop = p.drop(); L.poff = p.off; L.psc = p.sc; L.peps = p.eps; L.prelu = p.relu;
                    L.pY = p.Y; L.ldpy = p.ldy; L.pxhat = p.xhat; L.prstd = p.rstd;
                }
            }
            rc = sgcn::ce_impl(op.op == SGCN_OP_SOFTMAX_CE, ce.z, ce.ldz, ce.lab, ce.ldl, ce.n, ce.c, ce.dz, ce.lddz, ce.pred, ce.ldp,
                               ce.stats, ce.rowstat, stream, overlap, (hd || tail) ? &L : nullptr);
            head.on = false;
            break;
        }
        case SGCN_OP_ADAM:
        case SGCN_OP_ADAM_EMA: {
            const bool ema = op.op == SGCN_OP_ADAM_EMA;
            float* th = a.p<float>(); const float* g = a.p<const float>(); float* m = a.p<float>(); float* v = a.p<float>();
            float* avg = ema ? a.p<float>() : nullptr;
// ... 88 lines not shown
            rc = h16 ? sgcn_vr_aggregate_post_h16(arp, ac, av, n1, n0, d, h, mu, ldx, (const uint16_t*)H, ldh, ifi, s, oh, om, ldo, cvd,
                                                  concat, accP, stream)
                     : sgcn_vr_aggregate_post_f32(arp, ac, av, n1, n0, d, h, mu, ldx, (const float*)H, ldh, ifi, s, oh, om, ldo, cvd,
                                                  concat, accP, stream);
            break;
        }
        case SGCN_OP_GATHER_ROWS: {
            const float* in = a.p<const float>(); const int64_t ldi = a.next();
            const int32_t* r = a.p<const int32_t>(); const int32_t n = a.i(), d = a.i();
            float* out = a.p<float>(); const int64_t ldo = a.next();
            rc = sgcn_gather_rows_f32(in, ldi, r, n, d, out, ldo, stream);
            break;
        }
        case SGCN_OP_DROPOUT: {
            const float* x = a.p<const float>(); const int64_t ldx = a.next();
            const int32_t n = a.i(), d = a.i();
            a.drop(&dr);
            float* out = a.p<float>(); const int64_t ldo = a.next();
            rc = sgcn_dropout_f32(x, ldx, n, d, &dr, out, ldo, stream);
            break;
        }
        case SGCN_OP_L2_PENALTY: {
            const float* th = a.p<const float>(); const int64_t lo = a.next(), hi = a.next();
            const float wd = a.f();
            float* g = a.p<float>(); float* loss = a.p<float>();
            rc = sgcn_l2_penalty_f32(th, lo, hi, wd, g, loss, stream);
            break;
        }
        case SGCN_OP_MEMSET0:
        case SGCN_OP_AUX_MEMSET0: {
            void* p = a.p<void>(); const int64_t bytes = a.next();
            if (bytes > 0 && hipMemsetAsync(p, 0, (size_t)bytes, (hipStream_t)side) != hipSuccess)
                return sgcn::fail(SGCN_ERR_HIP, "step_run: hipMemsetAsync failed");
            if (op.op == SGCN_OP_AUX_MEMSET0 && side != stream) memset_on_aux = true;
            break;
        }
        case SGCN_OP_COPY2D: {
            void* dst = a.p<void>(); const int64_t ldd = a.next();
            const void* src = a.p<const void>(); const int64_t lds = a.next();
            const int64_t rows = a.next(), cols = a.next();
            if (rows > 0 && cols > 0 &&
                hipMemcpy2DAsync(dst, (size_t)ldd * 4, src, (size_t)lds * 4, (size_t)cols * 4, (size_t)rows,
                                 hipMemcpyDeviceToDevice, (hipStream_t)stream) != hipSuccess)
                return sgcn::fail(SGCN_ERR_HIP, "step_run: hipMemcpy2DAsync failed");
            break;
        }
        default:
            return sgcn::fail(SGCN_ERR_INVALID, "step_run: unknown opcode %d at op %d", op.op, k);
        }
        if (rc != SGCN_OK) { sgcn::aux_join(stream); xchg_join(stream); return rc; }
    }
    const int rj = sgcn::aux_join(stream);
    const int rx = xchg_join(stream);
    return rj != SGCN_OK ? rj : rx;
}
```

stochastic_gcn_amd/step_program.py:

```python
import ctypes as C

import numpy as np
import torch

from . import ops
from ._ffi import StepFill, StepOp, check, lib
from .flags import FLAGS
from .layers import AugmentedDropoutDense, Dense, DetDropoutFC, Dropout, PlainAggregator, VRAggregator
from .scheduler import CSR_DESC, PackedBatch

OP = dict(DENSE_FWD=1, DENSE_BWD=2, VR_AGG=3, SPMM=4, SOFTMAX_CE=5, ADAM=6, SCATTER_ROWS=7, MEMSET0=8,
          DROPOUT=9, L2_PENALTY=10, GATHER_ROWS=11, COPY2D=12, SIGMOID_CE=13, VR_AGG_PRE=14, VR_AGG_POST=15,
          AUX_SCATTER_ROWS=16, AUX_MEMSET0=17, DW_FLUSH=21, GRAD_STORE=22, MODE=23,
          CSR_SLICE=24, LN_ACT_FWD=25, LN_ACT_BWD=26, CSR_TRANSPOSE=27, GATHER_F32=28,
          ALLREDUCE_AVG=29, HIST_PACK=30, ALLGATHER_I32=31, HIST_APPLY=32,
          GEMM=33, DET_PRE=34, DET_PRE_BWD=35, SQUARE=36, ADDMUL=37, DET_LNVAR_FWD=38, DET_LNVAR_BWD=39, DET_RELU_FWD=40,
          DET_RELU_BWD=41, GAUSS=42, GAUSS_BWD=43, DET_AGG_PREP=44, DET_AGG_PREP_BWD=45, RELU_EPS=46, GATE=47,
          VR_AGG_H16=48, VR_AGG_PRE_H16=49, VR_AGG_POST_H16=50, SCATTER_ROWS_H16=51, AUX_SCATTER_ROWS_H16=52,
          HIST_APPLY_H16=53,
          ADAM_EMA=54)
MAX_ARGS = 48
GEMM_WS_BOUND = 256 * 32 * 128 + 64
ARENA_LIMIT_BYTES = 2 << 30

# ... 360 lines not shown
    def _sparse_bwd(self, g, rec):
        _, lay, xs, vals, y, ctx, relu, post = rec
        n, N = g.rows, g.cols
        if post:
            norm = ctx is not None
            need = (int(lib.sgcn_ln_act_bwd_ws_floats(n.cap, N)) + 3) // 4 * 4 if norm else 0
            self._ws_need = max(self._ws_need, need + GEMM_WS_BOUND)
            dx = self._alloc(n, N)
            self._emit('LN_ACT_BWD', [self._p(g), K(g.ld), self._p(y), K(y.ld), self._p(ctx[0]) if norm else NULL,
                                      self._p(ctx[1]) if norm else NULL, self._p(self._param(lay, 'scale')) if norm else NULL,
                                      n.op(), K(N), K(int(bool(relu))), self._p(dx), K(N),
                                      self._p(self._param(lay, 'offset', True)) if norm else NULL,
                                      self._p(self._param(lay, 'scale', True)) if norm else NULL,
                                      K(self._ws_gemm_ptr), K(self.gemm_ws_floats)])
            g = dx
        if xs.tbox[0] is None:
            ws_ints = int(lib.sgcn_csr_transpose_ws_ints(xs.ncols, xs.cap))
            trp, trow, tsrc = self._alloc_vec(xs.ncols + 1)[0], self._alloc_vec(xs.cap)[0], self._alloc_vec(xs.cap)[0]
            ws = self._alloc_vec(max(ws_ints, 1))[0]
            self._emit('CSR_TRANSPOSE', [K(xs.ncols), xs.nnz, xs.o_c, xs.o_r, trp, trow, tsrc, ws, K(ws_ints)])
            xs.tbox[0] = (trp, trow, tsrc)
        trp, trow, tsrc = xs.tbox[0]
        tv = self._alloc_vec(xs.cap)[0]
        self._emit('GATHER_F32', [vals, tsrc, xs.nnz, tv])
        dW = self._param(lay, 'weights', True)
        self._emit('SPMM', [trp, trow, tv, K(xs.ncols), n.op(), K(N), self._p(g), K(g.ld), NULL, NULL, NULL,
                            self._p(dW), K(dW.ld), K(_fbits(1.0)), K(0), NULL, K(0), NULL, K(0), K(0), NULL, K(0), NULL, K(0), K(0)])
        return None

    def _param(self, layer, name, grad=False):
        t = (layer.grads if grad else layer.vars).get(name)
        if t is None:
            return None
        rows, cols = int(t.shape[0]), int(t.shape[1])
        return ST(K(t.data_ptr()), Rows(0, -1, rows, rows), cols, cols)

    def _build(self):
        m = self.model
        F = m.features_dev
        if self.sparse:
            cap = max(self.nnz_cap, 1)
            o_p = self._alloc_vec(self.caps[0] + 1)[0]
            o_c, o_d, o_r = self._alloc_vec(cap)[0], self._alloc_vec(cap)[0], self._alloc_vec(cap)[0]
            act = SSparse(o_p, o_c, o_d, o_r, self.rows[0], self._nnz(), int(F.shape[1]), cap)
            self._emit('CSR_SLICE', [self.rows[0].op(), self._field_ptr(0), K(F.val.data_ptr()), K(F.col.data_ptr()),
                                     K(F.rowptr.data_ptr()), o_p, o_d, o_c, o_r])
        else:
            feat = ST(K(F.data_ptr()), Rows(0, -1, int(F.shape[0]), int(F.shape[0])), int(F.shape[1]), int(F.stride(0)))
            act = SGather(feat, self._field_ptr(0), self.rows[0])
        tape = []
        concat = FLAGS.normalization != 'gcn'
        self.new_history = {}
        self.overlap = int(bool(FLAGS.agg_overlap) or not (FLAGS.lean_sync and FLAGS.group_dw))
        self.native_world = int(getattr(m, 'native_coll', 0) or 0) if m.is_training else 0
        self.exchange_overlap = bool(self.native_world and getattr(getattr(m, '_par', None), 'exchange_overlap', False))
        self._exchanged = set()
        local_hist = m.history_hook is None and not self.native_world
        self._hist_last = bool(FLAGS.lean_sync) and local_hist
        self.det = bool(FLAGS.det_dropout)
        if self.det and (self.native_world or m.history_hook is not None):
            raise Unsupported("det-dropout with a multi-GPU history exchange")
        if m.is_training:
            if self.sparse or self.det:
                self._emit('MEMSET0', [K(m.grad.data_ptr()), K(m.grad.numel() * 4)])
            elif FLAGS.lean_sync:
                self._emit('GRAD_STORE', [])
            else:
                self._emit('AUX_MEMSET0', [K(m.grad.data_ptr()), K(m.grad.numel() * 4)])
        accP = {}
        two_phase = bool(FLAGS.agg_overlap) and not self.det
        for layer in m.layers:
            if two_phase and isinstance(layer, VRAggregator):
                l = layer.l
                bf = self._csr(l, 2)
                hist = m.history[l][0]
                d = int(hist.shape[1])
                ldw = (d + 3) // 4 * 4
                buf = self._alloc(self.rows[l + 1], ldw)
                self._emit(self._hop('VR_AGG_PRE', hist), [self._ip(bf + 3), self._ip(bf + 4), self._fp(bf + 5), self.rows[l + 1].op(), self._n(bf + 1),
                                          K(d), K(hist.data_ptr()), K(int(hist.stride(0))), self._ip(self._pb.o_ffields + 2 * l),
                                          self._p(buf)] + self._plan(bf, d))
                accP[l] = buf
        for layer in m.layers:
            if isinstance(layer, (AugmentedDropoutDense, Dense)) and layer.sparse_inputs:
                if not isinstance(act, SSparse):
                    raise Unsupported("sparse layer behind a dense activation")
                xs = act
                aug = isinstance(layer, AugmentedDropoutDense)
                site = self._site(layer) if aug else None
                W = self._param(layer, 'weights')
                off = self._param(layer, 'offset') if layer.norm else None
                sc = self._param(layer, 'scale') if layer.norm else None
                relu = True if aug else bool(layer.act)
                vals = xs.vals
                if site is not None:
                    vals = self._sparse_dropout(xs, site)
                hx, ctx = self._sparse_fwd(xs, vals, W, off, sc, relu, aug or layer.norm or layer.act)
                tape.append(('sdense', layer, xs, vals, hx, ctx, relu, aug or layer.norm or layer.act))
                if aug:
                    hmu = hx if site is None else self._sparse_fwd(xs, xs.vals, W, off, sc, True, True)[0]
                    act = (hx, hmu)
                else:
                    act = hx
            elif isinstance(layer, AugmentedDropoutDense):
                if layer.output_dim > 128:
                    raise Unsupported("wide AugmentedDropoutDense")
# ... 322 lines not shown
                    A2t = self._sq_vals(bt, self._nnz_cap(l, 1))
                    g_ds2, g_msig2 = self._alloc(n0, d), self._alloc(n0, d)
                    self._spmm(bt, gvg, g_ds2, d, vals=A2t)
                    self._spmm(bt, gvg, g_msig2, d, vals=self._fp(self._pb.o_tmedg + 2 * l))
                    d_var = self._alloc(n0, d)
                    addv = g[1].cols_from(0, d) if cc else None
                    self._emit('DET_AGG_PREP_BWD', [self._p(var), self._p(ds), self._p(sbar), self._p(g_ds2), self._p(g_msig2), n0.op(), K(d),
                                                    self._p(addv), K(addv.ld if addv is not None else 0), n1.op() if cc else K(0),
                                                    self._p(d_var)])
                    g = (d_mu, d_var)
                elif rec[0] == 'agg':
                    _, l, d, cc, sptr = rec
                    bt = self._csr(l, 1)
                    dx = self._alloc(self.rows[l], d)
                    if not cc:
                        self._spmm(bt, g, dx, d, cscale=sptr)
                    else:
                        self._spmm(bt, g.cols_from(d, d), dx, d, cscale=sptr, add=g.cols_from(0, d), add_rows=self.rows[l + 1].op())
                    g = dx
            if FLAGS.group_dw:
                self._emit('DW_FLUSH', [])
            if wd and hi > lo:
                self._emit('L2_PENALTY', [K(m.theta.data_ptr()), K(lo), K(hi), K(_fbits(wd)), K(m.grad.data_ptr()), NULL])
            if self.native_world:
                self._emit('ALLREDUCE_AVG', [K(m.grad.data_ptr()), K(m.grad.numel())])
            self._cur = self.ops_opt
            lr, betas = self._lr(), [K(_fbits(FLAGS.beta1)), K(_fbits(FLAGS.beta2)), K(_fbits(1e-8))]
            state = [K(m.theta.data_ptr()), K(m.grad.data_ptr()), K(m.adam_m.data_ptr()), K(m.adam_v.data_ptr())]
            avg = m.average
            if avg is None:
                self._emit('ADAM', state + [K(m.theta.numel()), lr] + betas)
            else:
                decay, one_minus = ops.polyak_factors(m.polyak_decay)
                self._emit('ADAM_EMA', state + [K(avg.data_ptr()), K(m.theta.numel()), lr] + betas +
                           [K(_fbits(decay)), K(_fbits(one_minus))])
        self._cur = self.ops_hist
        for l, nh in ({} if (local_hist and not self._hist_last) else self.new_history).items():
            if self.native_world:
                if l not in self._exchanged:
                    self._native_exchange(l, nh)
                continue
            for hist, src in zip(m.history[l], nh if isinstance(nh, list) else [nh]):
                self._emit(self._hop('SCATTER_ROWS', hist), [K(hist.data_ptr()), K(hist.stride(0)), self._field_ptr(l), self.rows[l].op(),
                                            K(src.cols), self._p(src), K(src.ld)])

    def _finalize(self):
        self._key_slots = {li: self._n_meta + i for i, li in enumerate(self._key_layers)}
        self.lr_slot = self._n_meta + len(self._key_layers)
        self.nnz_slot = self.lr_slot + 1
        self.nslots = self.lr_slot + (2 if self.sparse else 1)

        def pack(lst):
            if lst:
                lst = [(OP['MODE'], [K(self.overlap), K(-1)])] + list(lst)
            arr = (StepOp * max(len(lst), 1))()
            for k, (opc, args) in enumerate(lst):
                o = arr[k]
                o.op, o.nargs = opc, len(args)
                for j, a in enumerate(args):
                    o.mul[j], o.slot[j], o.add[j] = int(a[0]), int(a[1]), int(a[2])
            return arr
        self.c_fb, self.c_opt, self.c_hist = pack(self.ops_fb), pack(self.ops_opt), pack(self.ops_hist)
        self.n_fb, self.n_opt, self.n_hist = (len(x) + (1 if x else 0) for x in (self.ops_fb, self.ops_opt, self.ops_hist))
        allops = self.ops_fb + self.ops_opt + self.ops_hist
        self.c_all, self.n_all = pack(allops), len(allops) + (1 if allops else 0)
        f = np.array(self._fill, dtype=np.int64).reshape(-1, 3)
        self._f_idx, self._f_mul = f[:, 0].copy(), f[:, 1].copy()
        self._f_ip, self._f_fp = (f[:, 2] == 1).astype(np.int64), (f[:, 2] == 2).astype(np.int64)
        self.slots = np.zeros(self.nslots, dtype=np.int64)
        self._slots_ptr = self.slots.ctypes.data
        chk = np.array(self._cap_checks, dtype=np.int64).reshape(-1, 2)
        self._cap_idx, self._cap_max = chk[:, 0].copy(), chk[:, 1].copy()
        ns = np.array(self._nslot_checks, dtype=np.int64).reshape(-1, 2) if self._nslot_checks else np.zeros((0, 2), np.int64)
        self._ns_idx, self._ns_ldw = ns[:, 0].copy(), ns[:, 1].copy()
        so = self.stats_off
        self.loss_t, self.acc_t = self.arena[so + 2], self.arena[so + 3]
        self._keys = sorted(self._key_slots.items())
        self._f_base = f[:, 2].copy()
        self._key_slot = np.array([sl for _, sl in self._keys], dtype=np.int64)
        self._key_layer = np.array([li for li, _ in self._keys], dtype=np.int64)
        self._c_fill = StepFill(
            n=self._f_idx.shape[0], idx=self._f_idx.ctypes.data, mul=self._f_mul.ctypes.data, base=self._f_base.ctypes.data,
            n_cap=self._cap_idx.shape[0], cap_idx=self._cap_idx.ctypes.data, cap_max=self._cap_max.ctypes.data,
            n_ws=self._ns_idx.shape[0], ws_idx=self._ns_idx.ctypes.data, ws_ld=self._ns_ldw.ctypes.data,
            ws_floats=int(self.plan_ws_floats), n_keys=len(self._keys), key_slot=self._key_slot.ctypes.data,
            key_layer=self._key_layer.ctypes.data, lr_slot=self.lr_slot)
        self._c_fill_ref = C.byref(self._c_fill)
        self._runs = {'all': (self.c_all, self.n_all), 'fb': (self.c_fb, self.n_fb), 'opt': (self.c_opt, self.n_opt),
                      'hist': (self.c_hist, self.n_hist)}

    def fits(self, pb):
        meta = pb.meta
        if np.any(meta[self._cap_idx] > self._cap_max):
            return False
        if self._ns_idx.size and np.any(meta[self._ns_idx] * self._ns_ldw > self.plan_ws_floats):
            return False
        return True

    def fill(self, pb, ip, fp, step, lr_t):
        rc = lib.sgcn_step_fill(self._c_fill_ref, pb.meta_ptr, pb.meta.shape[0], ip, fp, self.model.dropout_seed, step, lr_t,
                                self._slots_ptr, self.nslots)
        if rc < 0:
            check(rc)
        if rc == 0 and self.sparse:
            m = pb.m
            nnz = int(self._rowlen[pb.ibuf[m[4]:m[4] + m[5]]].sum())
            if nnz > self.nnz_cap:
# ... 22 lines not shown
```

Measured before the change: 7.463 billion.

## Let VR aggregation history-part ride inside the preceding dense-forward GEMM

When a dense-forward pair is followed by a VR aggregation op, the step runner now records the aggregation's history (accP) SpMM so it can be computed alongside the dense GEMM. The later aggregation op then runs only a post kernel that consumes the precomputed accP. The aim is to hide the sparse history gather behind the GEMM and drop a separate launch. This adds scratch management, an abort path for when the GEMM does not take the ride, and a tune knob, agg_ride, whose default comes from sgcn_tune_get and the MODE op. A probe script for A/B testing is included.

```diff
diff --git a/include/sgcn.h b/include/sgcn.h
--- a/include/sgcn.h
+++ b/include/sgcn.h
@@ -135,6 +135,8 @@
 
 int sgcn_tune(const char* key, int64_t value);
 int64_t sgcn_tune_get(const char* key);
+int64_t sgcn_agg_ride_count(void);
+void sgcn_gemm_fwd_shape(int32_t M, int32_t N, int32_t K, int32_t* S, int32_t* kgroups, int32_t* kchunk);
 
 int sgcn_vr_aggregate_f32(const int32_t* dev_a_rowptr, const int32_t* dev_a_col,
                           const float* dev_a_val, const int32_t* dev_f_rowptr,
diff --git a/profiles/agg_ride_probe.py b/profiles/agg_ride_probe.py
--- /dev/null
+++ b/profiles/agg_ride_probe.py
@@ -0,0 +1,105 @@
+import argparse
+import json
+import os
+import statistics
+import subprocess
+import sys
+
+
+def _root(argv):
+    for i, a in enumerate(argv):
+        if a == "--root":
+            return os.path.abspath(argv[i + 1])
+    return os.path.dirname(os.path.dirname(os.path.abspath(__file__)))
+
+
+HERE = os.path.dirname(os.path.dirname(os.path.abspath(__file__)))
+ROOT = _root(sys.argv)
+sys.path.insert(0, ROOT)
+
+
+def epochs(args):
+    import torch
+    import bench
+    from stochastic_gcn_amd import _ffi, synthetic
+    has_knob = int(_ffi.lib.sgcn_tune_get(b"agg_ride")) >= 0
+    if args.ride >= 0:
+        if not has_knob:
+            raise SystemExit("this tree has no agg_ride knob")
+        _ffi.tune('agg_ride', args.ride)
+    dev = torch.device("cuda:0")
+    data = synthetic.reddit_like(seed=1, with_features=False)
+    err = sys.stderr
+    sys.stderr = open(os.devnull, "w") if args.quiet else err
+    try:
+        te = bench.train_epoch_leg(data, dev, epochs=args.epochs)
+    finally:
+        sys.stderr = err
+    rec = {"what": "epochs", "tree": "this commit" if ROOT == HERE else "parent (%s)" % os.path.basename(ROOT),
+           "agg_ride": int(_ffi.lib.sgcn_tune_get(b"agg_ride")) if has_knob else None,
+           "rides": int(_ffi.lib.sgcn_agg_ride_count()) if has_knob else None,
+           "epochs": args.epochs, "epoch_time_s": te["epoch_time_s"], "epoch_times_s": te["epoch_times_s"],
+           "ms_per_step": te["ms_per_step"], "steps": te["steps"], "gpu_chain_us": te.get("gpu_chain_us"),
+           "host_launch_us": te.get("host_launch_us"), "val_sweep_s": (te.get("validation") or {}).get("val_sweep_s"),
+           "ops_per_step": (te.get("chain_probe") or {}).get("ops_per_step")}
+    print(json.dumps(rec), flush=True)
+
+
+def _leg(r):
+    return "parent" if r["tree"].startswith("parent") else "ride%d" % r["agg_ride"]
+
+
+def verdict(rows):
+    for key in ("gpu_chain_us", "epoch_time_s", "val_sweep_s"):
+        col = lambda leg: [r[key] for r in rows if r.get("what") == "epochs" and _leg(r) == leg and r.get(key) is not None]
+        par, off, on = col("parent"), col("ride0"), col("ride1")
+        v = {"what": "verdict", "quantity": key, "parent": par, "ride0": off, "ride1": on}
+        if par:
+            v.update(parent_min=min(par), parent_max=max(par), parent_spread=max(par) - min(par))
+        if par and on:
+            v.update(ride1_worst=max(on), gain_worst_vs_parent_best=min(par) - max(on), ride1_worst_beats_parent_best=max(on) < min(par),
+                     median_gain=statistics.median(par) - statistics.median(on))
+        if par and off:
+            v["ride0_median_inside_parent_range"] = min(par) <= statistics.median(off) <= max(par)
+        print(json.dumps(v), flush=True)
+
+
+def cost(args):
+    legs = [("this", 0), ("this", 1)]
+    if args.parent:
+        legs.insert(0, ("parent", -1))
+    rows = []
+    for rep in range(args.repeats):
+        for tree, ride in legs:
+            cmd = [sys.executable, os.path.abspath(__file__), "epochs", "--ride", str(ride), "--epochs", str(args.epochs), "--quiet"]
+            if tree == "parent":
+                cmd += ["--root", os.path.abspath(args.parent)]
+            out = subprocess.run(cmd, stdout=subprocess.PIPE, cwd=os.path.abspath(args.parent) if tree == "parent" else HERE,
+                                 timeout=args.leg_timeout, check=True).stdout.decode()
+            rec = json.loads([l for l in out.splitlines() if l.startswith("{")][-1])
+            rec["repeat"] = rep
+            rows.append(rec)
+            print(json.dumps(rec), flush=True)
+    verdict(rows)
+
+
+def main():
+    ap = argparse.ArgumentParser()
+    ap.add_argument("what", choices=["epochs", "cost", "verdict"])
+    ap.add_argument("--ride", type=int, default=-1)
+    ap.add_argument("--epochs", type=int, default=8)
+    ap.add_argument("--repeats", type=int, default=3)
+    ap.add_argument("--parent", default=None, help="a checkout of the parent commit, built in its own tree")
+    ap.add_argument("--root", default=None)
+    ap.add_argument("--rows", default=None, help="verdict: a file of `epochs` rows")
+    ap.add_argument("--leg-timeout", type=int, default=300)
+    ap.add_argument("--quiet", action="store_true")
+    args = ap.parse_args()
+    if args.what == "verdict":
+        rows = [json.loads(l) for l in open(args.rows) if l.startswith("{")]
+        return verdict(rows)
+    {"epochs": epochs, "cost": cost}[args.what](args)
+
+
+if __name__ == "__main__":
+    main()
diff --git a/stochastic_gcn_amd/_ffi.py b/stochastic_gcn_amd/_ffi.py
--- a/stochastic_gcn_amd/_ffi.py
+++ b/stochastic_gcn_amd/_ffi.py
@@ -159,6 +159,8 @@
     "sgcn_ln_act_bwd_f32": (C.c_int, [P, C.c_int64, P, C.c_int64, P, P, P, C.c_int32, C.c_int32,
                                       C.c_int32, P, C.c_int64, P, P, P, P]),
     "sgcn_gemm_ws_floats": (C.c_int64, [C.c_int32, C.c_int32, C.c_int32]),
+    "sgcn_gemm_fwd_shape": (None, [C.c_int32, C.c_int32, C.c_int32, C.POINTER(C.c_int32), C.POINTER(C.c_int32), C.POINTER(C.c_int32)]),
+    "sgcn_agg_ride_count": (C.c_int64, []),
     "sgcn_gemm_f32": (C.c_int, [C.c_int32, C.c_int32, C.c_int32, C.c_int32, C.c_int32, P, C.c_int64, P,
                                 C.c_int64, P, C.c_int64, C.c_int32, P, P, P, P]),
     "sgcn_gemm_mb16_ws_floats": (C.c_int64, [C.c_int32, C.c_int32, C.c_int32, C.c_int32, C.c_int32]),
diff --git a/stochastic_gcn_amd/csrc/sgcn_agg.h b/stochastic_gcn_amd/csrc/sgcn_agg.h
--- /dev/null
+++ b/stochastic_gcn_amd/csrc/sgcn_agg.h
@@ -0,0 +1,195 @@
+#pragma once
+#include "sgcn_dev.h"
+#include "sgcn_fuse.h"
+#include <type_traits>
+
+namespace sgcn {
+
+
+template <int VW>
+__device__ __forceinline__ void store_masked(float* p, typename Vec<VW>::type v, int left) {
+    if (left >= VW) vstore<VW>(p, v);
+    else vstore_head<VW>(p, v, left);
+}
+
+template <int G, int VW, class HT>
+__device__ __forceinline__ void agg_apart(const AggArgsT<HT>& a, int row, int vi, int lig, bool act,
+                                          typename Vec<VW>::type& acc1, typename Vec<VW>::type& acc2) {
+    typedef typename Vec<VW>::type VT;
+    acc1 = vzero<VW>(); acc2 = vzero<VW>();
+    const int start = uniform_i<G>(a.a_rowptr[row]), end = uniform_i<G>(a.a_rowptr[row + 1]);
+    const int64_t voff = (int64_t)vi * VW;
+    for (int p0 = start; p0 < end; p0 += G) {
+        const int n = min(G, end - p0);
+        int mycol = 0, myhist = 0;
+        float myval = 0.f;
+        if (lig < n) {
+            mycol = a.a_col[p0 + lig];
+            myval = a.a_val[p0 + lig];
+            myhist = a.ifield[mycol];
+        }
+        for (int j = 0; j < n; j++) {
+            const int c = bcast_i<G>(mycol, j);
+            const int hr = bcast_i<G>(myhist, j);
+            const float v = bcast_f<G>(myval, j);
+            if (!act) continue;
+            const VT hb = hload<VW>(a.H + (int64_t)hr * a.ldh + voff);
+            const VT xv = vload<VW>(a.h + (int64_t)c * a.ldx + voff);
+            if constexpr (VW == 1 && !std::is_same<HT, float>::value) {
+                if (a.cvd) {
+                    const float mv = a.mu[(int64_t)c * a.ldx + voff];
+                    acc1 = __builtin_fmaf(v, mv - hb, acc1);
+                    acc2 = __builtin_fmaf(v, xv - mv, acc2);
+                } else {
+                    acc1 = __builtin_fmaf(v, xv, acc1);
+                    acc2 = __builtin_fmaf(v, hb, acc2);
+                }
+            } else if (a.cvd) {
+                const VT mv = vload<VW>(a.mu + (int64_t)c * a.ldx + voff);
+                acc1 += v * (mv - hb);
+                acc2 += v * (xv - mv);
+            } else {
+                acc1 += v * xv;
+                acc2 += v * hb;
+            }
+        }
+    }
+}
+
+template <int VW, class HT>
+__device__ __forceinline__ void agg_epilogue(const AggArgsT<HT>& a, int row, int vi, bool act, typename Vec<VW>::type accP,
+                                             typename Vec<VW>::type acc1, typename Vec<VW>::type acc2) {
+    typedef typename Vec<VW>::type VT;
+    if (!act) return;
+    const int64_t voff = (int64_t)vi * VW;
+    const int left = a.d - vi * VW;
+    float* oh = a.out_h + (int64_t)row * a.ldo;
+    if (a.cvd) {
+        float* om = a.out_mu + (int64_t)row * a.ldo;
+        const VT mu_nbr = acc1 + accP;
+        const VT h_nbr = acc2 * a.s[row] + mu_nbr;
+        store_masked<VW>(oh + a.off + voff, h_nbr, left);
+        store_masked<VW>(om + a.off + voff, mu_nbr, left);
+        if (a.concat) {
+            store_masked<VW>(oh + voff, vload<VW>(a.h + (int64_t)row * a.ldx + voff), left);
+            store_masked<VW>(om + voff, vload<VW>(a.mu + (int64_t)row * a.ldx + voff), left);
+        }
+    } else {
+        const VT out = (acc1 - acc2) + accP;
+        store_masked<VW>(oh + a.off + voff, out, left);
+        if (a.concat) store_masked<VW>(oh + voff, vload<VW>(a.h + (int64_t)row * a.ldx + voff), left);
+    }
+}
+
+template <int G, int VW, class HT>
+__device__ __forceinline__ void agg_finish(const AggArgsT<HT>& a, int row, int vi, int lig, bool act,
+                                           typename Vec<VW>::type accP) {
+    typename Vec<VW>::type acc1, acc2;
+    agg_apart<G, VW>(a, row, vi, lig, act, acc1, acc2);
+    agg_epilogue<VW>(a, row, vi, act, accP, acc1, acc2);
+}
+
+constexpr int agg_max_chunks(int G, int VW) { return (kBlock / G) * (4 / VW) - 1 < 31 ? (kBlock / G) * (4 / VW) - 1 : 31; }
+
+template <int G, int VW, int U, class HT, bool PONLY>
+__device__ __forceinline__ void agg_row_body(const AggArgsT<HT>& a, float (*part)[G * VW], const int tid, const int64_t blk,
+                                             const bool live) {
+    typedef typename Vec<VW>::type VT;
+    constexpr int NG = kBlock / G, NP = NG - 1;
+    constexpr int NC = agg_max_chunks(G, VW);
+    const int lig = tid & (G - 1), gq = tid / G;
+    int row = 0, start = 0, end = 0, slot = -1, vi = 0;
+    bool act = false;
+    const int nc = a.pchunks;
+    if (live) {
+        const int slab = (int)(blk / a.nseg);
+        const int64_t s = blk % a.nseg;
+        if (a.seg) {
+            const sgcn_seg_t sg = a.seg[s];
+            row = sg.row; start = sg.start; end = sg.end; slot = sg.slot;
+        } else {
+            row = (int)s; start = a.f_rowptr[s]; end = a.f_rowptr[s + 1]; slot = -1;
+        }
+        row = uniform_i<G>(row); start = uniform_i<G>(start);
+        end = uniform_i<G>(end); slot = uniform_i<G>(slot);
+        vi = slab * G + lig;
+        act = vi < a.nvec;
+        const bool finish_here = !PONLY && slot < 0 && !a.accP_out;
+        const HT* Hl = a.H + (int64_t)vi * VW;
+
+        if (gq < NP) {
+            const int chunk = (end - start + nc - 1) / nc;
+            for (int ck = gq; ck < nc; ck += NP) {
+                const int gs = start + ck * chunk, ge = min(end, gs + chunk);
+                VT accP = vzero<VW>();
+                for (int p0 = gs; p0 < ge; p0 += G) {
+                    const int n = min(G, ge - p0);
+                    int myrow = 0;
+                    float myval = 0.f;
+                    if (lig < n) {
+                        myrow = a.ffield[a.f_col[p0 + lig]];
+                        myval = a.f_val[p0 + lig];
+                    }
+                    hpin<HT, VW>(myrow); hpin<HT, VW>(myval);
+                    for (int j = 0; j < n; j += U) {
+                        typename HRaw<HT, VW>::type b[U];
+                        float v[U];
+#pragma unroll
+                        for (int u = 0; u < U; u++) {
+                            const bool in = j + u < n;
+                            const int c = bcast_i<G>(myrow, in ? j + u : 0);
+                            v[u] = in ? bcast_f<G>(myval, j + u) : 0.f;
+                            b[u] = (act && in) ? hraw<VW>(Hl + (int64_t)c * a.ldh) : hraw_zero<HT, VW>();
+                        }
+#pragma unroll
+                        for (int u = 0; u < U; u++) { hpin<HT, VW>(b[u]); accP += v[u] * hwiden<VW>(b[u]); }
+                    }
+                }
+                vstore<VW>(&part[ck][lig * VW], accP);
+            }
+        } else if (finish_here) {
+            if constexpr (!PONLY) {
+                VT acc1, acc2;
+                agg_apart<G, VW>(a, row, vi, lig, act, acc1, acc2);
+                vstore<VW>(&part[NC][lig * VW], acc1);
+                vstore<VW>(&part[NC + 1][lig * VW], acc2);
+            }
+        }
+    }
+    __syncthreads();
+    if (!live || gq != 0) return;
+    VT accP = vload<VW>(&part[0][lig * VW]);
+    if (nc == NP) {
+#pragma unroll
+        for (int q = 1; q < NP; q++) accP += vload<VW>(&part[q][lig * VW]);
+    } else {
+        for (int q = 1; q < nc; q++) accP += vload<VW>(&part[q][lig * VW]);
+    }
+    if (slot >= 0) { if (act) vstore<VW>(a.ws + (int64_t)slot * a.ldw + (int64_t)vi * VW, accP); }
+    else if (PONLY || a.accP_out) { if (act) vstore<VW>(a.accP_out + (int64_t)row * a.ldw + (int64_t)vi * VW, accP); }
+    else if constexpr (!PONLY) agg_epilogue<VW>(a, row, vi, act, accP, vload<VW>(&part[NC][lig * VW]), vload<VW>(&part[NC + 1][lig * VW]));
+}
+
+template <int G, int VW, class HT, bool PONLY>
+__device__ __forceinline__ void agg_fix_body(const AggArgsT<HT>& a, const sgcn_fix_t* fix, const int64_t nfix, const int64_t blk,
+                                             const int tid) {
+    typedef typename Vec<VW>::type VT;
+    constexpr int GPB = kBlock / G;
+    const int lig = tid & (G - 1);
+    const int64_t nfblk = (nfix + GPB - 1) / GPB;
+    const int slab = (int)(blk / nfblk);
+    const int64_t f = (blk % nfblk) * GPB + tid / G;
+    if (f >= nfix) return;
+    const sgcn_fix_t fx = fix[f];
+    const int vi = slab * G + lig;
+    const bool act = vi < a.nvec;
+    VT accP = vzero<VW>();
+    if (act) {
+        const float* w = a.ws + (int64_t)fx.first_slot * a.ldw + (int64_t)vi * VW;
+        for (int q = 0; q < fx.nslots; q++) accP += vload<VW>(w + (int64_t)q * a.ldw);
+    }
+    if (PONLY || a.accP_out) { if (act) vstore<VW>(a.accP_out + (int64_t)fx.row * a.ldw + (int64_t)vi * VW, accP); }
+    else if constexpr (!PONLY) agg_finish<G, VW>(a, uniform_i<G>(fx.row), vi, lig, act, accP);
+}
+
+}
diff --git a/stochastic_gcn_amd/csrc/sgcn_agg.hip b/stochastic_gcn_amd/csrc/sgcn_agg.hip
--- a/stochastic_gcn_amd/csrc/sgcn_agg.hip
+++ b/stochastic_gcn_amd/csrc/sgcn_agg.hip
@@ -1,209 +1,25 @@
-#include "sgcn_dev.h"
-#include <type_traits>
+#include "sgcn_agg.h"
+#include <algorithm>
 
 namespace sgcn {
 
 int group_lanes(int nvec);
 
-template <class HT>
-struct AggArgsT {
-    const int32_t* a_rowptr; const int32_t* a_col; const float* a_val;
-    const int32_t* f_rowptr; const int32_t* f_col; const float* f_val;
-    const sgcn_seg_t* seg; int64_t nseg; int64_t nsegblk;
-    const float* h; const float* mu; int64_t ldx;
-    const HT* H; int64_t ldh;
-    const int32_t* ifield; const int32_t* ffield; const float* s;
-    float* out_h; float* out_mu; int64_t ldo;
-    int32_t d, nvec, cvd, off, concat;
-    float* ws; int64_t ldw;
-    int32_t pchunks;
-    float* accP_out; const float* accP_in;
-};
-
-
-template <int VW>
-__device__ __forceinline__ void store_masked(float* p, typename Vec<VW>::type v, int left) {
-    if (left >= VW) vstore<VW>(p, v);
-    else vstore_head<VW>(p, v, left);
-}
-
-template <int G, int VW, class HT>
-__device__ __forceinline__ void agg_apart(const AggArgsT<HT>& a, int row, int vi, int lig, bool act,
-                                          typename Vec<VW>::type& acc1, typename Vec<VW>::type& acc2) {
-    typedef typename Vec<VW>::type VT;
-    acc1 = vzero<VW>(); acc2 = vzero<VW>();
-    const int start = uniform_i<G>(a.a_rowptr[row]), end = uniform_i<G>(a.a_rowptr[row + 1]);
-    const int64_t voff = (int64_t)vi * VW;
-    for (int p0 = start; p0 < end; p0 += G) {
-        const int n = min(G, end - p0);
-        int mycol = 0, myhist = 0;
-        float myval = 0.f;
-        if (lig < n) {
-            mycol = a.a_col[p0 + lig];
-            myval = a.a_val[p0 + lig];
-            myhist = a.ifield[mycol];
-        }
-        for (int j = 0; j < n; j++) {
-            const int c = bcast_i<G>(mycol, j);
-            const int hr = bcast_i<G>(myhist, j);
-            const float v = bcast_f<G>(myval, j);
-            if (!act) continue;
-            const VT hb = hload<VW>(a.H + (int64_t)hr * a.ldh + voff);
-            const VT xv = vload<VW>(a.h + (int64_t)c * a.ldx + voff);
-            if constexpr (VW == 1 && !std::is_same<HT, float>::value) {
-                if (a.cvd) {
-                    const float mv = a.mu[(int64_t)c * a.ldx + voff];
-                    acc1 = __builtin_fmaf(v, mv - hb, acc1);
-                    acc2 = __builtin_fmaf(v, xv - mv, acc2);
-                } else {
-                    acc1 = __builtin_fmaf(v, xv, acc1);
-                    acc2 = __builtin_fmaf(v, hb, acc2);
-                }
-            } else if (a.cvd) {
-                const VT mv = vload<VW>(a.mu + (int64_t)c * a.ldx + voff);
-                acc1 += v * (mv - hb);
-                acc2 += v * (xv - mv);
-            } else {
-                acc1 += v * xv;
-                acc2 += v * hb;
-            }
-        }
-    }
-}
-
-template <int VW, class HT>
-__device__ __forceinline__ void agg_epilogue(const AggArgsT<HT>& a, int row, int vi, bool act, typename Vec<VW>::type accP,
-                                             typename Vec<VW>::type acc1, typename Vec<VW>::type acc2) {
-    typedef typename Vec<VW>::type VT;
-    if (!act) return;
-    const int64_t voff = (int64_t)vi * VW;
-    const int left = a.d - vi * VW;
-    float* oh = a.out_h + (int64_t)row * a.ldo;
-    if (a.cvd) {
-        float* om = a.out_mu + (int64_t)row * a.ldo;
-        const VT mu_nbr = acc1 + accP;
-        const VT h_nbr = acc2 * a.s[row] + mu_nbr;
-        store_masked<VW>(oh + a.off + voff, h_nbr, left);
-        store_masked<VW>(om + a.off + voff, mu_nbr, left);
-        if (a.concat) {
-            store_masked<VW>(oh + voff, vload<VW>(a.h + (int64_t)row * a.ldx + voff), left);
-            store_masked<VW>(om + voff, vload<VW>(a.mu + (int64_t)row * a.ldx + voff), left);
-        }
-    } else {
-        const VT out = (acc1 - acc2) + accP;
-        store_masked<VW>(oh + a.off + voff, out, left);
-        if (a.concat) store_masked<VW>(oh + voff, vload<VW>(a.h + (int64_t)row * a.ldx + voff), left);
-    }
-}
-
-template <int G, int VW, class HT>
-__device__ __forceinline__ void agg_finish(const AggArgsT<HT>& a, int row, int vi, int lig, bool act,
-                                           typename Vec<VW>::type accP) {
-    typename Vec<VW>::type acc1, acc2;
-    agg_apart<G, VW>(a, row, vi, lig, act, acc1, acc2);
-    agg_epilogue<VW>(a, row, vi, act, accP, acc1, acc2);
-}
 
 static int p_chunks(int32_t d, const void* Hbar, int64_t ldh, const float* ws) {
     const int vw = pick_vw(d, {Hbar, ws}, {ldh, ((int64_t)d + 3) / 4 * 4});
     return kBlock / group_lanes((d + vw - 1) / vw) - 1;
 }
 
-constexpr int agg_max_chunks(int G, int VW) { return (kBlock / G) * (4 / VW) - 1 < 31 ? (kBlock / G) * (4 / VW) - 1 : 31; }
-
 template <int G, int VW, int U, class HT>
 __global__ __launch_bounds__(kBlock) void agg_row_kernel(AggArgsT<HT> a) {
-    typedef typename Vec<VW>::type VT;
-    constexpr int NG = kBlock / G, NP = NG - 1;
-    constexpr int NC = agg_max_chunks(G, VW);
-    __shared__ float part[NC + 2][G * VW];
-    const int lig = threadIdx.x & (G - 1), gq = threadIdx.x / G;
-    const int slab = (int)(blockIdx.x / a.nseg);
-    const int64_t s = blockIdx.x % a.nseg;
-    int row, start, end, slot;
-    if (a.seg) {
-        const sgcn_seg_t sg = a.seg[s];
-        row = sg.row; start = sg.start; end = sg.end; slot = sg.slot;
-    } else {
-        row = (int)s; start = a.f_rowptr[s]; end = a.f_rowptr[s + 1]; slot = -1;
-    }
-    row = uniform_i<G>(row); start = uniform_i<G>(start);
-    end = uniform_i<G>(end); slot = uniform_i<G>(slot);
-    const int vi = slab * G + lig;
-    const bool act = vi < a.nvec;
-    const bool finish_here = slot < 0 && !a.accP_out;
-    const HT* Hl = a.H + (int64_t)vi * VW;
-
-    const int nc = a.pchunks;
-    if (gq < NP) {
-        const int chunk = (end - start + nc - 1) / nc;
-        for (int ck = gq; ck < nc; ck += NP) {
-            const int gs = start + ck * chunk, ge = min(end, gs + chunk);
-            VT accP = vzero<VW>();
-            for (int p0 = gs; p0 < ge; p0 += G) {
-                const int n = min(G, ge - p0);
-                int myrow = 0;
-                float myval = 0.f;
-                if (lig < n) {
-                    myrow = a.ffield[a.f_col[p0 + lig]];
-                    myval = a.f_val[p0 + lig];
-                }
-                hpin<HT, VW>(myrow); hpin<HT, VW>(myval);
-                for (int j = 0; j < n; j += U) {
-                    typename HRaw<HT, VW>::type b[U];
-                    float v[U];
-#pragma unroll
-                    for (int u = 0; u < U; u++) {
-                        const bool in = j + u < n;
-                        const int c = bcast_i<G>(myrow, in ? j + u : 0);
-                        v[u] = in ? bcast_f<G>(myval, j + u) : 0.f;
-                        b[u] = (act && in) ? hraw<VW>(Hl + (int64_t)c * a.ldh) : hraw_zero<HT, VW>();
-                    }
-#pragma unroll
-                    for (int u = 0; u < U; u++) { hpin<HT, VW>(b[u]); accP += v[u] * hwiden<VW>(b[u]); }
-                }
-            }
-            vstore<VW>(&part[ck][lig * VW], accP);
-        }
-    } else if (finish_here) {
-        VT acc1, acc2;
-        agg_apart<G, VW>(a, row, vi, lig, act, acc1, acc2);
-        vstore<VW>(&part[NC][lig * VW], acc1);
-        vstore<VW>(&part[NC + 1][lig * VW], acc2);
-    }
-    __syncthreads();
-    if (gq != 0) return;
-    VT accP = vload<VW>(&part[0][lig * VW]);
-    if (nc == NP) {
-#pragma unroll
-        for (int q = 1; q < NP; q++) accP += vload<VW>(&part[q][lig * VW]);
-    } else {
-        for (int q = 1; q < nc; q++) accP += vload<VW>(&part[q][lig * VW]);
-    }
-    if (slot >= 0) { if (act) vstore<VW>(a.ws + (int64_t)slot * a.ldw + (int64_t)vi * VW, accP); }
-    else if (a.accP_out) { if (act) vstore<VW>(a.accP_out + (int64_t)row * a.ldw + (int64_t)vi * VW, accP); }
-    else agg_epilogue<VW>(a, row, vi, act, accP, vload<VW>(&part[NC][lig * VW]), vload<VW>(&part[NC + 1][lig * VW]));
+    __shared__ float part[agg_max_chunks(G, VW) + 2][G * VW];
+    agg_row_body<G, VW, U, HT, false>(a, part, (int)threadIdx.x, (int64_t)blockIdx.x, true);
 }
 
 template <int G, int VW, class HT>
 __global__ __launch_bounds__(kBlock) void agg_fix_kernel(AggArgsT<HT> a, const sgcn_fix_t* fix, int64_t nfix) {
-    typedef typename Vec<VW>::type VT;
-    constexpr int GPB = kBlock / G;
-    const int lig = threadIdx.x & (G - 1);
-    const int64_t nfblk = (nfix + GPB - 1) / GPB;
-    const int slab = (int)(blockIdx.x / nfblk);
-    const int64_t f = (blockIdx.x % nfblk) * GPB + threadIdx.x / G;
-    if (f >= nfix) return;
-    const sgcn_fix_t fx = fix[f];
-    const int vi = slab * G + lig;
-    const bool act = vi < a.nvec;
-    VT accP = vzero<VW>();
-    if (act) {
-        const float* w = a.ws + (int64_t)fx.first_slot * a.ldw + (int64_t)vi * VW;
-        for (int q = 0; q < fx.nslots; q++) accP += vload<VW>(w + (int64_t)q * a.ldw);
-    }
-    if (a.accP_out) { if (act) vstore<VW>(a.accP_out + (int64_t)fx.row * a.ldw + (int64_t)vi * VW, accP); }
-    else agg_finish<G, VW>(a, uniform_i<G>(fx.row), vi, lig, act, accP);
+    agg_fix_body<G, VW, HT, false>(a, fix, nfix, (int64_t)blockIdx.x, (int)threadIdx.x);
 }
 
 template <int G, int VW, class HT>
@@ -326,16 +142,17 @@
 }
 
 template <class HT>
-static int vr_aggregate_pre(const char* who, const int32_t* f_rowptr, const int32_t* f_col, const float* f_val, int32_t n1,
-                            int32_t nf, int32_t d, const HT* Hbar, int64_t ldh, const int32_t* ffield, float* accP,
-                            const sgcn_plan_t* f_plan, void* stream) {
+static int pre_args(const char* who, const int32_t* f_rowptr, const int32_t* f_col, const float* f_val, int32_t n1, int32_t nf,
+                    int32_t d, const HT* Hbar, int64_t ldh, const int32_t* ffield, float* accP, const sgcn_plan_t* f_plan,
+                    AggArgsT<HT>& a, int* vw_out, int* G_out) {
     constexpr bool kH16 = !std::is_same<HT, float>::value;
+    *vw_out = 0; *G_out = 0;
     SGCN_REQUIRE(n1 >= 0 && nf >= 0 && d >= 0, "%s: negative size", who);
     if constexpr (kH16) { if (int rc = h16_table_ok(who, Hbar, ldh, d)) return rc; }
     if (n1 == 0 || d == 0) return SGCN_OK;
     SGCN_REQUIRE(f_rowptr && Hbar && accP && ldh >= d, "%s: bad operand", who);
     SGCN_REQUIRE(nf == 0 || ffield, "%s: null ffield", who);
-    AggArgsT<HT> a{};
+    a = AggArgsT<HT>{};
     a.f_rowptr = f_rowptr; a.f_col = f_col; a.f_val = f_val;
     a.H = Hbar; a.ldh = ldh; a.ffield = ffield; a.d = d;
     a.ldw = ((int64_t)d + 3) / 4 * 4;
@@ -354,11 +171,77 @@
     const int G = group_lanes(a.nvec);
     a.pchunks = p_chunks(d, vw_table(Hbar), ldh, f_plan ? f_plan->dev_ws : nullptr);
     a.nsegblk = (a.nseg + (kBlock / G) - 1) / (kBlock / G);
+    *vw_out = vw; *G_out = G;
+    return SGCN_OK;
+}
+
+template <class HT>
+static int vr_aggregate_pre(const char* who, const int32_t* f_rowptr, const int32_t* f_col, const float* f_val, int32_t n1,
+                            int32_t nf, int32_t d, const HT* Hbar, int64_t ldh, const int32_t* ffield, float* accP,
+                            const sgcn_plan_t* f_plan, void* stream) {
+    AggArgsT<HT> a{};
+    int vw = 0, G = 0;
+    if (int rc = pre_args<HT>(who, f_rowptr, f_col, f_val, n1, nf, d, Hbar, ldh, ffield, accP, f_plan, a, &vw, &G)) return rc;
+    if (vw == 0) return SGCN_OK;
     hipStream_t st = (hipStream_t)stream;
     if (vw == 4) return launch_agg<4>(G, a, f_plan, st);
     if (vw == 2) return launch_agg<2>(G, a, f_plan, st);
     return launch_agg<1>(G, a, f_plan, st);
 }
+
+namespace sgcn {
+namespace {
+struct RideScratch { float* p = nullptr; int64_t cap = 0, want = 0; };
+RideScratch& ride_scratch() { static RideScratch s; return s; }
+int64_t g_ride_count = 0;
+}
+
+AggRide& agg_ride_state() { static AggRide r; return r; }
+void agg_ride_abort() { AggRide& r = agg_ride_state(); r.on = false; r.taken = false; }
+void agg_ride_count_one() { g_ride_count++; }
+
+float* agg_ride_scratch(int64_t floats) {
+    RideScratch& s = ride_scratch();
+    if (floats <= s.cap) return s.p;
+    s.want = std::max(s.want, floats);
+    return nullptr;
+}
+
+int agg_ride_scratch_grow(void* stream) {
+    RideScratch& s = ride_scratch();
+    if (s.want <= s.cap) return SGCN_OK;
+    SGCN_HIP_TRY(hipStreamSynchronize((hipStream_t)stream));
+    if (s.p) SGCN_HIP_TRY(hipFree(s.p));
+    s.p = nullptr; s.cap = 0;
+    const int64_t cap = s.want + s.want / 2;
+    SGCN_HIP_TRY(hipMalloc((void**)&s.p, (size_t)cap * sizeof(float)));
+    s.cap = cap; s.want = 0;
+    return SGCN_OK;
+}
+
+bool agg_ride_record(bool h16, const int32_t* f_rowptr, const int32_t* f_col, const float* f_val, int32_t n1, int32_t nf, int32_t d,
+                     const void* Hbar, int64_t ldh, const int32_t* ffield, float* accP, const sgcn_plan_t* f_plan) {
+    AggRide& r = agg_ride_state();
+    r = AggRide{};
+    int vw = 0, G = 0, rc;
+    if (h16) rc = pre_args<uint16_t>("agg_ride", f_rowptr, f_col, f_val, n1, nf, d, (const uint16_t*)Hbar, ldh, ffield, accP, f_plan, r.h, &vw, &G);
+    else rc = pre_args<float>("agg_ride", f_rowptr, f_col, f_val, n1, nf, d, (const float*)Hbar, ldh, ffield, accP, f_plan, r.f, &vw, &G);
+    const int pchunks = h16 ? r.h.pchunks : r.f.pchunks;
+    if (rc != SGCN_OK || vw != 4 || d % 4 != 0 || (G != 8 && G != 32) || pchunks < 1 || pchunks > agg_max_chunks(G, 4)) return false;
+    const int64_t nseg = h16 ? r.h.nseg : r.f.nseg;
+    const int nslab = ((h16 ? r.h.nvec : r.f.nvec) + G - 1) / G;
+    r.nblocks = nseg * nslab;
+    if (f_plan && f_plan->nfix > 0) {
+        r.fix = f_plan->dev_fix; r.nfix = f_plan->nfix;
+        r.nfixblk = (r.nfix + (kBlock / G) - 1) / (kBlock / G) * nslab;
+    }
+    if (r.nblocks <= 0 || r.nblocks >= (1ll << 30) || r.nfixblk >= (1ll << 30)) return false;
+    r.h16 = h16; r.G = G; r.on = true;
+    return true;
+}
+}
+
+extern "C" int64_t sgcn_agg_ride_count(void) { return sgcn::g_ride_count; }
 
 template <class HT>
 static int vr_aggregate_post(const char* who, const int32_t* a_rowptr, const int32_t* a_col, const float* a_val, int32_t n1,
diff --git a/stochastic_gcn_amd/csrc/sgcn_fuse.h b/stochastic_gcn_amd/csrc/sgcn_fuse.h
--- a/stochastic_gcn_amd/csrc/sgcn_fuse.h
+++ b/stochastic_gcn_amd/csrc/sgcn_fuse.h
@@ -15,4 +15,30 @@
     float* pY = nullptr; int64_t ldpy = 0; float* pxhat = nullptr; float* prstd = nullptr;
 };
 
+template <class HT>
+struct AggArgsT {
+    const int32_t* a_rowptr; const int32_t* a_col; const float* a_val;
+    const int32_t* f_rowptr; const int32_t* f_col; const float* f_val;
+    const sgcn_seg_t* seg; int64_t nseg; int64_t nsegblk;
+    const float* h; const float* mu; int64_t ldx;
+    const HT* H; int64_t ldh;
+    const int32_t* ifield; const int32_t* ffield; const float* s;
+    float* out_h; float* out_mu; int64_t ldo;
+    int32_t d, nvec, cvd, off, concat;
+    float* ws; int64_t ldw;
+    int32_t pchunks;
+    float* accP_out; const float* accP_in;
+};
+
+struct AggRide {
+    bool on = false;
+    bool taken = false;
+    bool h16 = false;
+    int32_t G = 0;
+    AggArgsT<float> f{};
+    AggArgsT<uint16_t> h{};
+    int64_t nblocks = 0;
+    const sgcn_fix_t* fix = nullptr; int64_t nfix = 0, nfixblk = 0;
+};
+
 }
diff --git a/stochastic_gcn_amd/csrc/sgcn_gemm.hip b/stochastic_gcn_amd/csrc/sgcn_gemm.hip
--- a/stochastic_gcn_amd/csrc/sgcn_gemm.hip
+++ b/stochastic_gcn_amd/csrc/sgcn_gemm.hip
@@ -1,5 +1,6 @@
 #include "sgcn_dev.h"
 #include "sgcn_bwd.h"
+#include "sgcn_agg.h"
 
 namespace sgcn {
 
@@ -227,6 +228,22 @@
     gemm_body<TA, TB, KG>(g, (int)blockIdx.x, (int)blockIdx.y, (int)blockIdx.z);
 }
 
+template <int KG, int G, int VW, class HT>
+__global__ __launch_bounds__(kBlock * KG) void gemm_ride_kernel(GemmArgs g, int32_t gx, int32_t gy, int32_t gemm_blocks,
+                                                                 AggArgsT<HT> a, int64_t nride) {
+    const int b = (int)blockIdx.x;
+    if (b < gemm_blocks) {
+        gemm_body<false, false, KG>(g, b % gx, (b / gx) % gy, b / (gx * gy));
+        return;
+    }
+    extern __shared__ __attribute__((aligned(16))) float ride_lds[];
+    static_assert((agg_max_chunks(G, VW) + 2) * G * VW <= kGroupFloats && kGroupFloats % 4 == 0, "a rider part fits a K-group's LDS");
+    const int part = (int)threadIdx.x / kBlock;
+    const int64_t blk = (int64_t)(b - gemm_blocks) * KG + part;
+    agg_row_body<G, VW, 16, HT, true>(a, reinterpret_cast<float (*)[G * VW]>(ride_lds + part * kGroupFloats), (int)threadIdx.x % kBlock,
+                                      blk, blk < nride);
+}
+
 struct GemmGroup {
     GemmArgs g[kMaxGroup];
     int32_t first[kMaxGroup + 1];
@@ -332,7 +349,7 @@
     float* Y; int64_t ldy; float* xhat; float* rstd;
 };
 
-__global__ __launch_bounds__(kBlock) void splitk_ln_dense_kernel(const float* __restrict__ ws, int32_t S, GemmArgs g, RowDense d) {
+__device__ __forceinline__ void splitk_ln_dense_body(const float* __restrict__ ws, const int32_t S, const GemmArgs& g, const RowDense& d) {
     extern __shared__ __attribute__((aligned(1024))) float wl[];
     const int lane = threadIdx.x & 63;
     const int64_t row = (int64_t)blockIdx.x * (kBlock / kWave) + threadIdx.x / kWave;
@@ -455,6 +472,18 @@
             y2[c] = d.relu ? fmaxf(y, 0.f) : y;
         }
     }
+}
+
+__global__ __launch_bounds__(kBlock) void splitk_ln_dense_kernel(const float* __restrict__ ws, int32_t S, GemmArgs g, RowDense d) {
+    splitk_ln_dense_body(ws, S, g, d);
+}
+
+template <int G, int VW, class HT>
+__global__ __launch_bounds__(kBlock) void splitk_ln_dense_ride_kernel(const float* __restrict__ ws, int32_t S, GemmArgs g, RowDense d,
+                                                                       int32_t row_blocks, AggArgsT<HT> a, const sgcn_fix_t* fix,
+                                                                       int64_t nfix) {
+    if ((int)blockIdx.x < row_blocks) { splitk_ln_dense_body(ws, S, g, d); return; }
+    agg_fix_body<G, VW, HT, true>(a, fix, nfix, (int64_t)blockIdx.x - row_blocks, (int)threadIdx.x);
 }
 
 }
@@ -548,6 +577,14 @@
     return SGCN_OK;
 }
 
+extern "C" void sgcn_gemm_fwd_shape(int32_t M, int32_t N, int32_t K, int32_t* S, int32_t* kgroups, int32_t* kchunk) {
+    int s = 1, kg = 1, kc = 0;
+    if (M > 0 && N > 0 && K >= 0) sgcn::gemm_fwd_shape(M, N, K, &s, &kg, &kc);
+    if (S) *S = s;
+    if (kgroups) *kgroups = kg;
+    if (kchunk) *kchunk = kc;
+}
+
 extern "C" int64_t sgcn_gemm_ws_floats(int32_t M, int32_t N, int32_t K) {
     if (M <= 0 || N <= 0 || K <= 0) return 0;
     const int S = split_factor(M, N, K);
@@ -572,6 +609,37 @@
     return launch_gemm(g, trans_a, trans_b, ws, (hipStream_t)stream);
 }
 
+
+namespace sgcn {
+AggRide& agg_ride_state();
+void agg_ride_count_one();
+}
+template <int KG, int G, class HT>
+static void launch_ride_gemm_one(const GemmArgs& g, const GemmPlan& p, const AggArgsT<HT>& a, int64_t nride, hipStream_t st) {
+    const int tiles = (int)(p.grid.x * p.grid.y * p.grid.z);
+    const unsigned riders = (unsigned)((nride + KG - 1) / KG);
+    hipLaunchKernelGGL((gemm_ride_kernel<KG, G, 4, HT>), dim3((unsigned)tiles + riders), dim3(kBlock * KG),
+                       (size_t)KG * kGroupFloats * sizeof(float), st, g, (int32_t)p.grid.x, (int32_t)p.grid.y, (int32_t)tiles, a, nride);
+}
+template <int KG, class HT>
+static void launch_ride_gemm_g(const GemmArgs& g, const GemmPlan& p, const AggArgsT<HT>& a, const AggRide& r, hipStream_t st) {
+    if (r.G == 8) launch_ride_gemm_one<KG, 8, HT>(g, p, a, r.nblocks, st);
+    else launch_ride_gemm_one<KG, 32, HT>(g, p, a, r.nblocks, st);
+}
+static void launch_ride_gemm(const GemmArgs& g, const GemmPlan& p, const AggRide& r, hipStream_t st) {
+    if (p.kgroups == 2) { if (r.h16) launch_ride_gemm_g<2, uint16_t>(g, p, r.h, r, st); else launch_ride_gemm_g<2, float>(g, p, r.f, r, st); }
+    else                { if (r.h16) launch_ride_gemm_g<1, uint16_t>(g, p, r.h, r, st); else launch_ride_gemm_g<1, float>(g, p, r.f, r, st); }
+}
+template <int G, class HT>
+static void launch_ride_rows_one(const GemmArgs& g, int S, const RowDense& d, unsigned rb, size_t lds, const AggArgsT<HT>& a,
+                                 const AggRide& r, hipStream_t st) {
+    hipLaunchKernelGGL((splitk_ln_dense_ride_kernel<G, 4, HT>), dim3(rb + (unsigned)r.nfixblk), dim3(kBlock), lds, st, g.ws, S, g, d,
+                       (int32_t)rb, a, r.fix, r.nfix);
+}
+static void launch_ride_rows(const GemmArgs& g, int S, const RowDense& d, unsigned rb, size_t lds, const AggRide& r, hipStream_t st) {
+    if (r.G == 8) { if (r.h16) launch_ride_rows_one<8, uint16_t>(g, S, d, rb, lds, r.h, r, st); else launch_ride_rows_one<8, float>(g, S, d, rb, lds, r.f, r, st); }
+    else          { if (r.h16) launch_ride_rows_one<32, uint16_t>(g, S, d, rb, lds, r.h, r, st); else launch_ride_rows_one<32, float>(g, S, d, rb, lds, r.f, r, st); }
+}
 
 namespace sgcn {
 int dense_fwd_pair(int32_t M, int32_t N, int32_t K, const float* X, int64_t ldx, const float* X2, int64_t ldx2, int32_t split,
@@ -603,11 +671,20 @@
     SGCN_REQUIRE(!d.drop.on || d.drop.width == N, "dense_fwd: the second layer's dropout width must be its input width");
     d.Y = Y2; d.ldy = ldy2; d.xhat = xhat2; d.rstd = rstd2;
     hipStream_t st = (hipStream_t)stream;
-    launch_prepared(g, p, 0, 0, st);
+    AggRide& ride = agg_ride_state();
+    const unsigned rb = (unsigned)((g.M + (kBlock / kWave) - 1) / (kBlock / kWave));
+    const int64_t tiles = (int64_t)p.grid.x * p.grid.y * p.grid.z;
+    const bool riding = ride.on && (p.kgroups == 1 || p.kgroups == 2) &&
+                        tiles + (ride.nblocks + p.kgroups - 1) / p.kgroups < (1ll << 31) && (int64_t)rb + ride.nfixblk < (1ll << 31);
+    ride.on = false;
+    if (riding) launch_ride_gemm(g, p, ride, st);
+    else launch_prepared(g, p, 0, 0, st);
     g.epi = p.epi;
-    const unsigned rb = (unsigned)((g.M + (kBlock / kWave) - 1) / (kBlock / kWave));
-    hipLaunchKernelGGL(splitk_ln_dense_kernel, dim3(rb), dim3(kBlock), ((size_t)N * N2 + 255) / 256 * 256 * sizeof(float), st, g.ws, p.S, g, d);
+    const size_t lds2 = ((size_t)N * N2 + 255) / 256 * 256 * sizeof(float);
+    if (riding && ride.nfix > 0) launch_ride_rows(g, p.S, d, rb, lds2, ride, st);
+    else hipLaunchKernelGGL(splitk_ln_dense_kernel, dim3(rb), dim3(kBlock), lds2, st, g.ws, p.S, g, d);
     SGCN_HIP_TRY(hipGetLastError());
+    if (riding) { ride.taken = true; agg_ride_count_one(); }
     *fused = 1;
     return SGCN_OK;
 }
diff --git a/stochastic_gcn_amd/csrc/sgcn_spmm.hip b/stochastic_gcn_amd/csrc/sgcn_spmm.hip
--- a/stochastic_gcn_amd/csrc/sgcn_spmm.hip
+++ b/stochastic_gcn_amd/csrc/sgcn_spmm.hip
@@ -14,6 +14,7 @@
 int g_tune_cs_noextra = 0;
 int g_tune_step_overlap = 1;
 int g_tune_step_fuse = 127;
+int g_tune_agg_ride = 0;
 int g_tune_cs_g2_wide = 0;
 int g_tune_cs_nowarp = 0;
 int g_tune_cs_last_pct = 80;
@@ -38,6 +39,7 @@
     if (!strcmp(key, "cs_noextra")) return g_tune_cs_noextra;
     if (!strcmp(key, "step_overlap")) return tl_step_overlap >= 0 ? tl_step_overlap : g_tune_step_overlap;
     if (!strcmp(key, "step_fuse")) return tl_step_fuse >= 0 ? tl_step_fuse : g_tune_step_fuse;
+    if (!strcmp(key, "agg_ride")) return g_tune_agg_ride;
     if (!strcmp(key, "cs_g2_wide")) return g_tune_cs_g2_wide;
     if (!strcmp(key, "cs_nowarp")) return g_tune_cs_nowarp;
     if (!strcmp(key, "cs_last_pct")) return g_tune_cs_last_pct;
@@ -276,6 +278,7 @@
     if (!strcmp(key, "cs_noextra")) { g_tune_cs_noextra = value != 0; return SGCN_OK; }
     if (!strcmp(key, "step_overlap")) { g_tune_step_overlap = value != 0; return SGCN_OK; }
     if (!strcmp(key, "step_fuse")) { SGCN_REQUIRE(value >= 0 && value <= 127, "step_fuse in 0..127"); g_tune_step_fuse = (int)value; return SGCN_OK; }
+    if (!strcmp(key, "agg_ride")) { SGCN_REQUIRE(value == 0 || value == 1, "agg_ride in {0,1}"); g_tune_agg_ride = (int)value; return SGCN_OK; }
     if (!strcmp(key, "cs_g2_wide")) { g_tune_cs_g2_wide = value != 0; return SGCN_OK; }
     if (!strcmp(key, "cs_nowarp")) { g_tune_cs_nowarp = value != 0; return SGCN_OK; }
     if (!strcmp(key, "gemm_min_steps")) { g_tune_gemm_min_steps = (int)value; return SGCN_OK; }
diff --git a/stochastic_gcn_amd/csrc/sgcn_step.cpp b/stochastic_gcn_amd/csrc/sgcn_step.cpp
--- a/stochastic_gcn_amd/csrc/sgcn_step.cpp
+++ b/stochastic_gcn_amd/csrc/sgcn_step.cpp
@@ -43,6 +43,12 @@
                    const int32_t* gidx2, int32_t N2, const float* W2, int64_t ldw2, const float* offset2, const float* scale2,
                    float eps2, int32_t relu2, float* Y2, int64_t ldy2, float* xhat2, float* rstd2, const sgcn_dropout_t* drop2,
                    void* stream, int* fused);
+AggRide& agg_ride_state();
+bool agg_ride_record(bool h16, const int32_t* f_rowptr, const int32_t* f_col, const float* f_val, int32_t n1, int32_t nf, int32_t d,
+                     const void* Hbar, int64_t ldh, const int32_t* ffield, float* accP, const sgcn_plan_t* f_plan);
+void agg_ride_abort();
+float* agg_ride_scratch(int64_t floats);
+int agg_ride_scratch_grow(void* stream);
 }
 
 namespace {
@@ -112,6 +118,24 @@
     }
     const sgcn_dropout_t* drop() const { return has_drop ? &dr : nullptr; }
 };
+struct VrAggOp {
+    const int32_t *arp, *ac, *frp, *fc, *ifi, *ffi; const float *av, *fv, *h, *mu, *s; const void* H;
+    int32_t n1, n0, nf, d, cvd, concat; int64_t ldx, ldh, ldo; float *oh, *om;
+    sgcn_plan_t pl; bool has_plan;
+    void read(Args& a) {
+        arp = a.p<const int32_t>(); ac = a.p<const int32_t>(); av = a.p<const float>();
+        frp = a.p<const int32_t>(); fc = a.p<const int32_t>(); fv = a.p<const float>();
+        n1 = a.i(); n0 = a.i(); nf = a.i(); d = a.i();
+        h = a.p<const float>(); mu = a.p<const float>(); ldx = a.next();
+        H = a.p<const void>(); ldh = a.next();
+        ifi = a.p<const int32_t>(); ffi = a.p<const int32_t>();
+        s = a.p<const float>();
+        oh = a.p<float>(); om = a.p<float>(); ldo = a.next();
+        cvd = a.i(); concat = a.i();
+        has_plan = a.plan(&pl) != nullptr;
+    }
+    const sgcn_plan_t* plan() const { return has_plan ? &pl : nullptr; }
+};
 struct CeOp {
     const float *z, *lab; int64_t ldz, ldl, lddz, ldp; int32_t n, c; float *dz, *pred, *stats, *rowstat;
     void read(Args& a) {
@@ -259,13 +283,14 @@
     static std::mutex run_mutex;
     std::lock_guard<std::mutex> run_lock(run_mutex);
     bool memset_on_aux = false;
-    int64_t run_overlap = sgcn_tune_get("step_overlap"), run_fuse = sgcn_tune_get("step_fuse");
+    int64_t run_overlap = sgcn_tune_get("step_overlap"), run_fuse = sgcn_tune_get("step_fuse"), run_ride = sgcn_tune_get("agg_ride");
     bool own_mode = false;
     for (int32_t k = 0; k < nops; k++)
         if (ops[k].op == SGCN_OP_MODE && ops[k].nargs >= 1) {
             own_mode = true;
             run_overlap = ops[k].add[0] != 0;
             if (ops[k].nargs >= 2 && ops[k].add[1] >= 0) run_fuse = ops[k].add[1] & 127;
+            if (ops[k].nargs >= 3 && ops[k].add[2] >= 0) run_ride = ops[k].add[2] != 0;
         }
     const bool overlap = run_overlap != 0;
     const int fuse = (int)run_fuse;
@@ -289,7 +314,7 @@
     sgcn::stats_defer(park_stats ? 1 : 0);
     struct Guard {
         bool on; void* st;
-        ~Guard() { if (on) sgcn::dw_group_abort(); sgcn::grad_store_mode(0); sgcn::stats_defer(0); sgcn::reduce_flush(st); sgcn::stats_flush(st); }
+        ~Guard() { if (on) sgcn::dw_group_abort(); sgcn::agg_ride_abort(); sgcn::grad_store_mode(0); sgcn::stats_defer(0); sgcn::reduce_flush(st); sgcn::stats_flush(st); }
     } guard{grouped, stream};
     auto eval_args = [&](const sgcn_step_op_t& o, Args& a) {
         a.n = o.nargs; a.pos = 0;
@@ -301,6 +326,8 @@
         return true;
     };
     int32_t skip_until = 0, dx_done_at = -1;
+    int32_t ride_at = -1;
+    const float* ride_accP = nullptr;
     struct Head { bool on = false, pre = false; int32_t at = -1, kg = 1, pS = 1, pkchunk = 0, pkg = 1; DenseFwdOp f, p; } head;
     auto peek = [&](int32_t j, Args& b) {
         return j < nops && ops[j].nargs >= 0 && ops[j].nargs <= SGCN_STEP_MAX_ARGS && eval_args(ops[j], b);
@@ -381,10 +408,24 @@
                                    (!q.X2 || (q.X2 == f.Y + (int64_t)q.split * f.ldy && q.ldx2 == f.ldy)) &&
                                    (!q.has_drop || q.dr.rows == q.split || !q.X2);
                 if (whole) {
+                    int32_t j = k + 2;
+                    while (j < nops && ops[j].op == SGCN_OP_DENSE_FWD) j++;
+                    Args c;
+                    if (run_ride && ride_at < 0 && j < nops && f32_op(ops[j].op) == SGCN_OP_VR_AGG && peek(j, c)) {
+                        VrAggOp v;
+                        v.read(c);
+                        float* accP = (v.n1 > 0 && v.d > 0) ? sgcn::agg_ride_scratch((int64_t)v.n1 * (((int64_t)v.d + 3) / 4 * 4)) : nullptr;
+                        if (accP && sgcn::agg_ride_record(ops[j].op != SGCN_OP_VR_AGG, v.frp, v.fc, v.fv, v.n1, v.nf, v.d, v.H, v.ldh, v.ffi,
+                                                          accP, v.plan())) {
+                            ride_at = j; ride_accP = accP;
+                        }
+                    }
                     int fusedq = 0;
                     rc = sgcn::dense_fwd_pair(f.M, f.N, f.K, f.X, f.ldx, f.X2, f.ldx2, f.split, f.W, f.ldw, f.off, f.sc, f.eps, f.relu,
                                               f.Y, f.ldy, f.xhat, f.rstd, f.drop(), f.ws, f.g1, f.g2, q.N, q.W, q.ldw, q.off, q.sc, q.eps,
                                               q.relu, q.Y, q.ldy, q.xhat, q.rstd, q.drop(), stream, &fusedq);
+                    if (!sgcn::agg_ride_state().taken) { sgcn::agg_ride_abort(); ride_at = -1; }
+                    sgcn::agg_ride_state().taken = false;
                     if (rc != SGCN_OK) break;
                     if (fusedq) { skip_until = k + 2; break; }
                 }
@@ -575,20 +616,20 @@
         }
         case SGCN_OP_VR_AGG:
         case SGCN_OP_VR_AGG_H16: {
-            const int32_t* arp = a.p<const int32_t>(); const int32_t* ac = a.p<const int32_t>(); const float* av = a.p<const float>();
-            const int32_t* frp = a.p<const int32_t>(); const int32_t* fc = a.p<const int32_t>(); const float* fv = a.p<const float>();
-            const int32_t n1 = a.i(), n0 = a.i(), nf = a.i(), d = a.i();
-            const float* h = a.p<const float>(); const float* mu = a.p<const float>(); const int64_t ldx = a.next();
-            const void* H = a.p<const void>(); const int64_t ldh = a.next();
-            const int32_t* ifi = a.p<const int32_t>(); const int32_t* ffi = a.p<const int32_t>();
-            const float* s = a.p<const float>();
-            float* oh = a.p<float>(); float* om = a.p<float>(); const int64_t ldo = a.next();
-            const int32_t cvd = a.i(), concat = a.i();
-            const sgcn_plan_t* p = a.plan(&pl);
-            rc = h16 ? sgcn_vr_aggregate_h16(arp, ac, av, frp, fc, fv, n1, n0, nf, d, h, mu, ldx, (const uint16_t*)H, ldh, ifi, ffi,
-                                             s, oh, om, ldo, cvd, concat, p, stream)
-                     : sgcn_vr_aggregate_f32(arp, ac, av, frp, fc, fv, n1, n0, nf, d, h, mu, ldx, (const float*)H, ldh, ifi, ffi,
-                                             s, oh, om, ldo, cvd, concat, p, stream);
+            VrAggOp v;
+            v.read(a);
+            if (k == ride_at) {
+                rc = h16 ? sgcn_vr_aggregate_post_h16(v.arp, v.ac, v.av, v.n1, v.n0, v.d, v.h, v.mu, v.ldx, (const uint16_t*)v.H, v.ldh,
+                                                      v.ifi, v.s, v.oh, v.om, v.ldo, v.cvd, v.concat, ride_accP, stream)
+                         : sgcn_vr_aggregate_post_f32(v.arp, v.ac, v.av, v.n1, v.n0, v.d, v.h, v.mu, v.ldx, (const float*)v.H, v.ldh,
+                                                      v.ifi, v.s, v.oh, v.om, v.ldo, v.cvd, v.concat, ride_accP, stream);
+                ride_at = -1;
+                break;
+            }
+            rc = h16 ? sgcn_vr_aggregate_h16(v.arp, v.ac, v.av, v.frp, v.fc, v.fv, v.n1, v.n0, v.nf, v.d, v.h, v.mu, v.ldx,
+                                             (const uint16_t*)v.H, v.ldh, v.ifi, v.ffi, v.s, v.oh, v.om, v.ldo, v.cvd, v.concat, v.plan(), stream)
+                     : sgcn_vr_aggregate_f32(v.arp, v.ac, v.av, v.frp, v.fc, v.fv, v.n1, v.n0, v.nf, v.d, v.h, v.mu, v.ldx,
+                                             (const float*)v.H, v.ldh, v.ifi, v.ffi, v.s, v.oh, v.om, v.ldo, v.cvd, v.concat, v.plan(), stream);
             break;
         }
         case SGCN_OP_SPMM: {
@@ -783,5 +824,6 @@
     }
     const int rj = sgcn::aux_join(stream);
     const int rx = xchg_join(stream);
-    return rj != SGCN_OK ? rj : rx;
-}
+    const int rg = sgcn::agg_ride_scratch_grow(stream);
+    return rj != SGCN_OK ? rj : rx != SGCN_OK ? rx : rg;
+}
diff --git a/stochastic_gcn_amd/step_program.py b/stochastic_gcn_amd/step_program.py
--- a/stochastic_gcn_amd/step_program.py
+++ b/stochastic_gcn_amd/step_program.py
@@ -436,6 +436,7 @@
         concat = FLAGS.normalization != 'gcn'
         self.new_history = {}
         self.overlap = int(bool(FLAGS.agg_overlap) or not (FLAGS.lean_sync and FLAGS.group_dw))
+        self.agg_ride = -1
         self.native_world = int(getattr(m, 'native_coll', 0) or 0) if m.is_training else 0
         self.exchange_overlap = bool(self.native_world and getattr(getattr(m, '_par', None), 'exchange_overlap', False))
         self._exchanged = set()
@@ -864,7 +865,7 @@
 
         def pack(lst):
             if lst:
-                lst = [(OP['MODE'], [K(self.overlap), K(-1)])] + list(lst)
+                lst = [(OP['MODE'], [K(self.overlap), K(-1), K(self.agg_ride)])] + list(lst)
             arr = (StepOp * max(len(lst), 1))()
             for k, (opc, args) in enumerate(lst):
                 o = arr[k]
```

Result: slower. 7.379 billion (-1.1%).
